# azmyrajab/polars_ols

Measured on AMD Instinct MI355X. Metric: group_regressions_per_sec, higher is better.
Workload: dtype f32

## Files before the change

### polars_ols_amd/csrc/api.hip

```cpp
#include <algorithm>
#include <cmath>
#include <cctype>
#include <cstdlib>
#include <strings.h>
#include <condition_variable>
#include <mutex>
#include <thread>

#include "common.hpp"
#include "api_internal.hpp"
#include "k1_gram_chol.hpp"
#include "k2_resident.hpp"
#include "k2w_resident.hpp"
#include "k3_rls.hpp"
#include "k4_rolling.hpp"
#include "k5_enet.hpp"
#include "k6_svd.hpp"
#include "k7_stats.hpp"
#include "k7r_robust.hpp"
#include "k7c_cluster.hpp"
#include "k7i_influence.hpp"
#include "k8_wide.hpp"
#include "k10_ridge_path.hpp"
#include "k11_rlm.hpp"
#include "k13_glm.hpp"
#include "k14_iv.hpp"
#include "k12_enet_cv.hpp"
#include "dyn_prep.hpp"

namespace pols {
template <typename T> bool k1m_fits(int k_user, bool has_w, int64_t max_rows);

__global__ void __launch_bounds__(256) mark_fallback_kernel(const int64_t *offs, int64_t n_groups, int32_t *status, int32_t *fb_flag,
                                                            int32_t epoch, int only_if_not_empty) {
    const int64_t g = (int64_t)blockIdx.x * 256 + threadIdx.x;
    if (g == 0) *fb_flag = epoch;
    if (g >= n_groups) return;
    if (only_if_not_empty) { if (status[g] != POLS_GROUP_EMPTY) status[g] = POLS_GROUP_FALLBACK; }
    else status[g] = POLS_GROUP_FALLBACK;
    (void)offs;
}

static thread_local char g_err[512] = "";

void set_error(const char *fmt, ...) {
    va_list ap;
    va_start(ap, fmt);
    vsnprintf(g_err, sizeof(g_err), fmt, ap);
    va_end(ap);
}

int fail(int code, const char *fmt, ...) {
    va_list ap;
    va_start(ap, fmt);
    vsnprintf(g_err, sizeof(g_err), fmt, ap);
    va_end(ap);
    return code;
}

int grow(DeviceBuffer &b, size_t bytes, void **out, bool *fresh) {
    if (fresh) *fresh = bytes > b.cap;
    if (bytes > b.cap) {
        if (b.ptr) POLS_HIP(hipFree(b.ptr));
        b.ptr = nullptr;
        b.cap = 0;
        const size_t want = std::max(bytes, (size_t)1 << 16);
        POLS_HIP(hipMalloc(&b.ptr, want));
        b.cap = want;
    }
    *out = b.ptr;
    return POLS_OK;
}
int grow(CachedTable &t, size_t bytes, void **out) {
    if (bytes > t.buf.cap) t.valid = false;
    return grow(t.buf, bytes, out);
}
int ensure_scratch(pols_ctx *ctx, Work w, size_t bytes, void **out) { return grow(ctx->work[(int)w], bytes, out); }

int upload_small(pols_ctx *ctx, void *dst_device, const void *src, size_t bytes) {
    if (bytes == 0) return POLS_OK;
    if (bytes > ((size_t)1 << 20)) {
        POLS_HIP(hipMemcpyAsync(dst_device, src, bytes, hipMemcpyHostToDevice, ctx->stream));
        POLS_HIP(hipStreamSynchronize(ctx->stream));
        return POLS_OK;
    }
    auto &slot = ctx->pinned[ctx->pinned_next];
    ctx->pinned_next = (ctx->pinned_next + 1) % 4;
    if (slot.busy) { POLS_HIP(hipEventSynchronize(slot.done)); slot.busy = false; }
    if (bytes > slot.cap) {
        if (slot.ptr) POLS_HIP(hipHostFree(slot.ptr));
        slot.ptr = nullptr; slot.cap = 0;
        const size_t want = std::max(bytes, (size_t)1 << 16);
        POLS_HIP(hipHostMalloc(&slot.ptr, want, hipHostMallocDefault));
        slot.cap = want;
    }
    if (!slot.done) POLS_HIP(hipEventCreateWithFlags(&slot.done, hipEventDisableTiming));
    std::memcpy(slot.ptr, src, bytes);
    POLS_HIP(hipMemcpyAsync(dst_device, slot.ptr, bytes, hipMemcpyHostToDevice, ctx->stream));
    POLS_HIP(hipEventRecord(slot.done, ctx->stream));
    slot.busy = true;
    return POLS_OK;
}

int upload_offsets(pols_ctx *ctx, const int64_t *offs, int64_t n_groups, const int64_t **d_offs, int64_t *max_rows,
                   uint64_t generation) {
    const int64_t cnt = n_groups + 1;
    const size_t bytes = sizeof(int64_t) * (size_t)cnt;
    if (generation != 0 && ctx->offsets.valid && ctx->offs_host == offs && ctx->offs_n == n_groups &&
        ctx->offs_generation == generation) {
        *d_offs = static_cast<const int64_t *>(ctx->offsets.buf.ptr);
        *max_rows = ctx->offs_max_rows;
        return POLS_OK;
    }
    uint64_t h0 = 1469598103934665603ULL, h1 = 0x9E3779B97F4A7C15ULL, h2 = 0xC2B2AE3D27D4EB4FULL, h3 = 0x165667B19E3779F9ULL;
    const uint64_t P = 1099511628211ULL;
    const uint64_t *u = reinterpret_cast<const uint64_t *>(offs);
    int64_t g = 0;
    for (; g + 4 <= cnt; g += 4) {
        h0 = (h0 ^ u[g]) * P; h1 = (h1 ^ u[g + 1]) * P; h2 = (h2 ^ u[g + 2]) * P; h3 = (h3 ^ u[g + 3]) * P;
    }
    for (; g < cnt; ++g) h0 = (h0 ^ u[g]) * P;
    int64_t mx = 0, ored = 0, mn = 0, mn_pos = INT64_MAX;
    for (int64_t i = 0; i < cnt; ++i) ored |= offs[i];
    int32_t small_mask = 0;
    int64_t hist_cnt[48] = {0}, hist_rows[48] = {0};
    int64_t over = 0;
    for (int64_t i = 1; i < cnt; ++i) {
        const int64_t d = offs[i] - offs[i - 1];
        mn = d < mn ? d : mn; mx = d > mx ? d : mx;
        mn_pos = (d > 0 && d < mn_pos) ? d : mn_pos;
        over += d > 1021 ? d - 1021 : 0;
        if (d > 0 && d <= 32) small_mask |= d <= 4 ? 1 : (d <= 8 ? 2 : (d <= 16 ? 4 : 8));
        const int bkt = d <= 1 ? 0 : 64 - __builtin_clzll((unsigned long long)(d - 1));
        hist_cnt[bkt < 47 ? bkt : 47]++; hist_rows[bkt < 47 ? bkt : 47] += d;
    }
    if (mn < 0) return fail(POLS_ERR_INVALID, "group_offsets must be ascending");
    const uint64_t sum = ((h0 * 31 + h1) * 31 + h2) * 31 + h3;
    const bool hit = ctx->offsets.valid && ctx->offs_n == n_groups && ctx->offs_sum == sum &&
                     ctx->offs_copy.size() == (size_t)cnt && std::memcmp(ctx->offs_copy.data(), offs, bytes) == 0;
    if (!hit) {
        void *dptr = nullptr;
        ctx->offsets.valid = false;
        int rc = grow(ctx->offsets, bytes, &dptr);
        if (rc) return rc;
        if ((rc = upload_small(ctx, dptr, offs, bytes))) return rc;
        ctx->offsets.valid = true;
        ctx->offs_copy.assign(offs, offs + cnt);
        ctx->offs_n = n_groups;
        ctx->offs_sum = sum;
        ctx->offs_id++;
    }
    ctx->offs_host = offs;
    ctx->offs_generation = generation;
    ctx->offs_max_rows = mx;
    ctx->offs_min_rows = mn_pos == INT64_MAX ? 0 : mn_pos;
    ctx->offs_small_mask = small_mask;
    std::memcpy(ctx->offs_hist_cnt, hist_cnt, sizeof(hist_cnt));
    std::memcpy(ctx->offs_hist_rows, hist_rows, sizeof(hist_rows));
    ctx->offs_wave_overflow = over;
    {
        int64_t tail = -1;
        for (int64_t i = n_groups; i >= 1; --i)
            if (offs[i] > offs[i - 1]) { tail = i - 1; break; }
        ctx->offs_tail_group = tail;
    }
    ctx->offs_aligned[0] = (ored & 1) == 0;
    ctx->offs_aligned[1] = (ored & 3) == 0;
    *d_offs = static_cast<const int64_t *>(ctx->offsets.buf.ptr);
    *max_rows = mx;
    return POLS_OK;
}

static bool ieq(const char *a, const char *b) {
    for (; *a && *b; ++a, ++b)
        if (std::tolower((unsigned char)*a) != std::tolower((unsigned char)*b)) return false;
    return *a == *b;
}

bool options_set(Options &o, const char *key, const char *v) {
    if (!key) return false;
    if (!strncasecmp(key, "POLS_", 5)) key += 5;
    const bool on = v != nullptr;
    const Options d;
    if (ieq(key, "TIMELINE")) o.timeline = on;
    else if (ieq(key, "K1_NOOCC4")) o.k1_noocc4 = on;
    else if (ieq(key, "K1_NOFAST")) o.k1_nofast = on;
    else if (ieq(key, "K1_NOEDGE")) o.k1_noedge = on;
    else if (ieq(key, "K1_NOTINY")) o.k1_notiny = on;
    else if (ieq(key, "K1_NORC1")) o.k1_norc1 = on;
    else if (ieq(key, "K1_SHAPE")) { o.k1_shape_team = on && ieq(v, "team"); o.k1_shape_wave = on && ieq(v, "wave"); }
    else if (ieq(key, "K1_F64_TEAM")) o.k1_f64_team256 = on && std::atoi(v) == 256;
    else if (ieq(key, "KG_NOYV")) o.kg_noyv = on;
    else if (ieq(key, "KG_SINGLE_BUFFER")) o.kg_single_buffer = on;
    else if (ieq(key, "NO_CLASSES")) o.no_classes = on;
    else if (ieq(key, "PREDICT_LOOP")) o.predict_loop = on;
    else if (ieq(key, "K2_NOPREFETCH")) o.k2_noprefetch = on;
    else if (ieq(key, "NO_SPLIT")) o.no_split = on;
    else if (ieq(key, "K1_PASSES")) o.k1_passes = on ? std::atoi(v) : d.k1_passes;
    else if (ieq(key, "K1_WG")) o.k1_wg = on ? std::atoi(v) : d.k1_wg;
    else if (ieq(key, "K1T_RC4")) o.k1t_rc4 = on ? (std::atoi(v) != 0) : d.k1t_rc4;
    else if (ieq(key, "K1T_SUB8")) o.k1t_sub8 = on ? std::atoi(v) : d.k1t_sub8;
    else if (ieq(key, "K1_NT_LOADS")) o.k1_nt_loads = on ? (std::atoi(v) != 0) : d.k1_nt_loads;
    else if (ieq(key, "K1_XCD")) o.k1_xcd = on ? std::atoi(v) : d.k1_xcd;
    else if (ieq(key, "K4P_LPS")) o.k4p_lps = on ? std::atoi(v) : d.k4p_lps;
    else if (ieq(key, "SEG_TARGET")) o.seg_target = on ? std::atoi(v) : d.seg_target;
    else if (ieq(key, "K1_RC2_WIDE")) o.k1_rc2_wide = on ? std::atoi(v) != 0 : d.k1_rc2_wide;
    else if (ieq(key, "DEBUG_SKIP_FIXUP")) o.debug_skip_fixup = on && std::atoi(v) != 0;
    else if (ieq(key, "K1_PERSIST")) o.k1_persist = on ? (std::atoi(v) != 0) : d.k1_persist;
    else if (ieq(key, "K1_PERSIST_SUB")) o.k1_persist_sub = on ? std::atoi(v) : d.k1_persist_sub;
    else if (ieq(key, "K1T_SUB32")) o.k1t_sub32 = on ? (std::atoi(v) != 0) : d.k1t_sub32;
    else if (ieq(key, "STATIC_ENGINE")) o.static_engine = !on ? 0 : ieq(v, "stream") ? 1 : ieq(v, "k2") ? 2 : ieq(v, "nok2") ? 3 : ieq(v, "k2w") ? 4 : 0;
    else if (ieq(key, "RLS_ENGINE")) o.rls_engine = !on ? 0 : ieq(v, "seq") ? 1 : ieq(v, "scan") ? 2 : ieq(v, "chunk") ? 3 : ieq(v, "halo") ? 4 : 0;
    else if (ieq(key, "RLM_ENGINE")) o.rlm_engine = !on ? 0 : ieq(v, "stream") ? 1 : 0;
    else if (ieq(key, "GLM_ENGINE")) o.glm_engine = !on ? 0 : ieq(v, "split") ? 1 : 0;
    else if (ieq(key, "RLS_SPINS")) o.rls_spin_limit = on ? std::atoi(v) : d.rls_spin_limit;
    else if (ieq(key, "RLS_EARLY")) o.rls_early = on ? std::atoi(v) : d.rls_early;
    else if (ieq(key, "ROLLING_ENGINE")) o.rolling_engine = !on ? 0 : ieq(v, "chunk") ? 1 : ieq(v, "halo") ? 2 : ieq(v, "nocompact") ? 3 : ieq(v, "halowave") ? 4 : ieq(v, "scatter") ? 5 : 0;
    else if (ieq(key, "K1_ENGINE")) o.k1_engine = !on ? 0 : ieq(v, "valu") ? 1 : ieq(v, "mfma") ? 2 : 0;
    else if (ieq(key, "K9_TAKE")) o.k9_take = !on ? 0 : ieq(v, "gather") ? 1 : ieq(v, "scatter") ? 2 : 0;
    else return false;
    return true;
}

void options_from_env(Options &o) {
    static const char *const keys[] = {"TIMELINE", "K1_NOOCC4", "K1_NOFAST", "K1_NOTINY", "K1_NORC1", "K1_SHAPE", "K1_F64_TEAM",
                                       "KG_NOYV", "K2_NOPREFETCH", "K1_PASSES", "K1_WG", "RLS_SPINS", "RLS_EARLY", "K1T_RC4", "K1_NT_LOADS", "STATIC_ENGINE",
                                       "RLS_ENGINE", "RLM_ENGINE", "GLM_ENGINE", "ROLLING_ENGINE", "K1_ENGINE", "K9_TAKE", "K1_PERSIST", "K1_PERSIST_SUB", "K1T_SUB32", "K1_NOEDGE", "K1T_SUB8",
                                       "K1_XCD", "NO_SPLIT", "DEBUG_SKIP_FIXUP", "K4P_LPS", "SEG_TARGET", "K1_RC2_WIDE", "KG_SINGLE_BUFFER", "PREDICT_LOOP", "NO_CLASSES"};
    char name[64];
    for (const char *k : keys) {
        std::snprintf(name, sizeof(name), "POLS_%s", k);
        if (const char *v = std::getenv(name)) options_set(o, k, v);
    }
}

static bool timing_sampled(pols_ctx *ctx) {
    if (!ctx->timing) return false;
    return (ctx->timing_tick++ % ctx->timing_stride) == 0;
}

void timing_begin(pols_ctx *ctx) {
    ctx->timing_open = false;
    if (!timing_sampled(ctx)) return;
    ctx->timing_open = true;
    if (ctx->timed_used == ctx->timed.size()) {
        TimedLaunch t;
        if (hipEventCreate(&t.start) != hipSuccess || hipEventCreate(&t.stop) != hipSuccess) return;
        ctx->timed.push_back(t);
    }
    hipEventRecord(ctx->timed[ctx->timed_used].start, ctx->stream);
}

bool timing_pair(pols_ctx *ctx, hipEvent_t *start, hipEvent_t *stop) {
    if (!timing_sampled(ctx)) return false;
    if (ctx->timed_used == ctx->timed.size()) {
        TimedLaunch t;
        if (hipEventCreate(&t.start) != hipSuccess || hipEventCreate(&t.stop) != hipSuccess) return false;
        ctx->timed.push_back(t);
    }
    *start = ctx->timed[ctx->timed_used].start;
    *stop = ctx->timed[ctx->timed_used].stop;
    ctx->timed_used++;
    return true;
}

void timing_end(pols_ctx *ctx) {
    if (!ctx->timing_open || ctx->timed_used >= ctx->timed.size()) return;
    ctx->timing_open = false;
    hipEventRecord(ctx->timed[ctx->timed_used].stop, ctx->stream);
    ctx->timed_used++;
}

int check_ctx(pols_ctx *ctx) {
    if (!ctx) return fail(POLS_ERR_INVALID, "ctx is NULL");
    POLS_HIP(hipSetDevice(ctx->device));
    return POLS_OK;
}


template <typename T>
__global__ void __launch_bounds__(256) null_weights_kernel(const T *w, T *out, int64_t n) {
    using V = typename Vec16<T>::type;
    constexpr int VN = Vec16<T>::N;
    const int64_t i0 = ((int64_t)blockIdx.x * 256 + threadIdx.x) * VN;
    if (i0 + VN <= n) {
        const V v = *reinterpret_cast<const V *>(w + i0);
        T f[4];
#pragma unroll
        for (int e = 0; e < VN; ++e) { const T x = vget<T>(v, e); f[e] = x != x ? (T)1e-24 : x; }
        if constexpr (VN == 4) *reinterpret_cast<V *>(out + i0) = V{f[0], f[1], f[2], f[3]};
        else *reinterpret_cast<V *>(out + i0) = V{f[0], f[1]};
    } else {
        for (int64_t i = i0; i < n; ++i) { const T x = w[i]; out[i] = x != x ? (T)1e-24 : x; }
    }
}

int fill_null_weights(pols_ctx *ctx, const pols_batch *b, Staged *st) {
    if (!st->w || b->null_free || b->n_rows <= 0) return POLS_OK;
    void *dst = const_cast<void *>(st->w);
    if (b->mem == POLS_MEM_DEVICE) {
        int rc = ensure_scratch(ctx, Work::NullWeights, round256(dtype_size(b->dtype) * (size_t)b->n_rows), &dst);
        if (rc) return rc;
    }
    const int vn = b->dtype == POLS_F32 ? 4 : 2;
    const unsigned blocks = (unsigned)((b->n_rows + 256 * (int64_t)vn - 1) / (256 * (int64_t)vn));
    if (b->dtype == POLS_F32) hipLaunchKernelGGL(null_weights_kernel<float>, dim3(blocks), dim3(256), 0, ctx->stream, static_cast<const float *>(st->w), static_cast<float *>(dst), b->n_rows);
    else hipLaunchKernelGGL(null_weights_kernel<double>, dim3(blocks), dim3(256), 0, ctx->stream, static_cast<const double *>(st->w), static_cast<double *>(dst), b->n_rows);
    POLS_HIP(hipGetLastError());
    st->w = dst;
    return POLS_OK;
}

int stage_inputs(pols_ctx *ctx, const pols_batch *b, int64_t coef_rows, int kt, const pols_out *o, Staged *st) {
    const size_t sz = dtype_size(b->dtype);
    const size_t colb = round256(sz * (size_t)b->n_rows);
    st->x.assign((size_t)b->n_features, nullptr);
    if (b->mem == POLS_MEM_DEVICE) {
        st->y = b->y; st->w = b->weights; st->valid = b->valid;
        for (int j = 0; j < b->n_features; ++j) st->x[j] = b->x_cols[j];
        if (o) { st->coef = o->coef; st->pred = o->pred; st->resid = o->resid; st->status = o->status; }
        bool ok = aligned16(st->y) && aligned16(st->w) && aligned16(st->pred) && aligned16(st->resid);
        for (int j = 0; j < b->n_features; ++j) ok = ok && aligned16(st->x[j]);
        if (!ok) return fail(POLS_ERR_INVALID, "device columns must be 16-byte aligned");
        return POLS_OK;
    }
    const int ncols = b->n_features + 1 + (b->weights ? 1 : 0);
    void *in = nullptr, *out = nullptr;
    int rc = ensure_scratch(ctx, Work::HostInputs, colb * ncols + round256((size_t)b->n_rows), &in);
    if (rc) return rc;
    char *p = static_cast<char *>(in);
    auto put = [&](const void *src, size_t bytes, const void **dst) -> int {
        POLS_HIP(hipMemcpyAsync(p, src, bytes, hipMemcpyHostToDevice, ctx->stream));
        *dst = p;
        p += round256(bytes);
        return POLS_OK;
    };
    if ((rc = put(b->y, sz * b->n_rows, &st->y))) return rc;
    for (int j = 0; j < b->n_features; ++j)
        if ((rc = put(b->x_cols[j], sz * b->n_rows, &st->x[j]))) return rc;
    if (b->weights && (rc = put(b->weights, sz * b->n_rows, &st->w))) return rc;
    if (b->valid) {
        const void *v = nullptr;
        if ((rc = put(b->valid, (size_t)b->n_rows, &v))) return rc;
        st->valid = static_cast<const uint8_t *>(v);
    }
    if (o) {
        const size_t coefb = round256(sz * (size_t)coef_rows * kt);
        const size_t statb = round256(sizeof(int32_t) * (size_t)b->n_groups);
        rc = ensure_scratch(ctx, Work::HostOutputs, coefb + 2 * colb + statb, &out);
        if (rc) return rc;
        char *q = static_cast<char *>(out);
        if (o->coef) st->coef = q;
        q += coefb;
        if (o->pred) st->pred = q;
        q += colb;
        if (o->resid) st->resid = q;
        q += colb;
        if (o->status) st->status = reinterpret_cast<int32_t *>(q);
    }
    return POLS_OK;
}

int unstage_outputs(pols_ctx *ctx, const pols_batch *b, int64_t coef_rows, int kt, const pols_out *o, const Staged &st) {
    if (b->mem == POLS_MEM_DEVICE) return POLS_OK;
    const size_t sz = dtype_size(b->dtype);
    if (o->coef) POLS_HIP(hipMemcpyAsync(o->coef, st.coef, sz * (size_t)coef_rows * kt, hipMemcpyDeviceToHost, ctx->stream));
    if (o->pred) POLS_HIP(hipMemcpyAsync(o->pred, st.pred, sz * (size_t)b->n_rows, hipMemcpyDeviceToHost, ctx->stream));
    if (o->resid) POLS_HIP(hipMemcpyAsync(o->resid, st.resid, sz * (size_t)b->n_rows, hipMemcpyDeviceToHost, ctx->stream));
    if (o->status) POLS_HIP(hipMemcpyAsync(o->status, st.status, sizeof(int32_t) * (size_t)b->n_groups, hipMemcpyDeviceToHost, ctx->stream));
    POLS_HIP(hipStreamSynchronize(ctx->stream));
    return POLS_OK;
}

int check_batch(const pols_batch *b, const pols_out *o, int max_features) {
    if (!b || !o) return fail(POLS_ERR_INVALID, "batch / out is NULL");
    if (b->dtype != POLS_F32 && b->dtype != POLS_F64) return fail(POLS_ERR_INVALID, "dtype must be POLS_F32 or POLS_F64");
    if (b->mem != POLS_MEM_HOST && b->mem != POLS_MEM_DEVICE) return fail(POLS_ERR_INVALID, "mem must be POLS_MEM_HOST or POLS_MEM_DEVICE");
    if (b->n_rows < 0 || b->n_groups < 0) return fail(POLS_ERR_INVALID, "negative size");
    if (b->n_features < 1) return fail(POLS_ERR_INVALID, "must pass at least 2 series");
    if (b->n_features + (b->add_intercept ? 1 : 0) > max_features)
        return fail(POLS_ERR_UNSUPPORTED, "%d features (+ intercept) > %d", b->n_features, max_features);
    if (!b->group_offsets || !b->x_cols || (!b->y && b->n_rows)) return fail(POLS_ERR_INVALID, "NULL column / offsets pointer");
    if (b->group_offsets[0] != 0 || b->group_offsets[b->n_groups] != b->n_rows)
        return fail(POLS_ERR_INVALID, "group_offsets must start at 0 and end at n_rows");
    for (int j = 0; j < b->n_features; ++j)
        if (!b->x_cols[j] && b->n_rows) return fail(POLS_ERR_INVALID, "x_cols[%d] is NULL", j);
    return POLS_OK;
}

static bool k1_valu_takes(const pols_ctx *ctx, bool f32, int kt, int64_t max_rows, bool has_w = false) {
    const int vec = f32 ? 4 : 2;
    if (kt <= 8 && max_rows <= (int64_t)256 * 2 * vec) return true;
    const int64_t need = max_rows + (ctx->offs_aligned[f32 ? 1 : 0] ? 0 : vec - 1);
    if (kt <= K1_MAX_KT && ctx->opt.static_engine != 2) {
        if (kt <= 8 || (ctx->opt.k1_rc2_wide && !(!f32 && kt == 10 && has_w))) return need <= (int64_t)256 * 4 * vec;
        return need <= 1024;
    }
    if (kt <= K1_MAX_KT) return need <= 1024;
    if (kt <= K1W_MAX_KT) return need <= (int64_t)256 * 2 * vec;
    if (!f32 && kt == 16 && need <= 16 * vec && !ctx->opt.k1_notiny) return true;
    if (!f32 && (kt < 17 || kt > 24)) return false;
    return kt <= K1X_MAX_KT && need <= (int64_t)256 * 1 * vec;
}
static bool k1_nulls_takes(const pols_ctx *ctx, bool f32, int kt, int64_t max_rows) {
    const int vec = f32 ? 4 : 2;
    if (kt <= 8 && max_rows <= (int64_t)256 * 2 * vec) return true;
    const int64_t need = max_rows + (ctx->offs_aligned[f32 ? 1 : 0] ? 0 : vec - 1);
    if (kt <= K1_MAX_KT) return need <= 1024;
    if (kt <= K1W_MAX_KT) return need <= (int64_t)256 * 2 * vec;
    if (!f32 && (kt < 17 || kt > 24)) return false;
    return kt <= K1X_MAX_KT && need <= (int64_t)256 * 1 * vec;
}

struct Compacted {
    pols_batch bb;
    std::vector<int64_t> offs;
    std::vector<const void *> xcols, ycols;
    Staged st;
    const int64_t *d_offs = nullptr;
    const uint8_t *vbytes = nullptr;
    RowCompactArgs ra;
};

static int compact_nulls(pols_ctx *ctx, const pols_batch *b, int policy, Compacted *c, const void *const *targets = nullptr,
                         int n_targets = 0) {
    int rc;
    const int64_t *d_offs = nullptr;
    int64_t max_rows = 0;
    Staged &st = c->st;
    if ((rc = upload_offsets(ctx, b->group_offsets, b->n_groups, &d_offs, &max_rows, b->offsets_generation))) return rc;
    if ((rc = stage_inputs(ctx, b, 0, 0, nullptr, &st))) return rc;
    const int m = n_targets > 0 ? n_targets : 1;
    const int k = b->n_features, ncols = m + k + (st.w ? 1 : 0);
    const size_t G = (size_t)b->n_groups, N = (size_t)b->n_rows;
    const size_t sz = dtype_size(b->dtype), colb = round256(sz * std::max<size_t>(N, 1));
    const size_t n_slabs = (N + 255) / 256;
    const size_t vb = round256(std::max<size_t>(N, 1)), tabb = round256(sizeof(void *) * (size_t)ncols), offb = round256(sizeof(int64_t) * (G + 1));
    const size_t cntb = round256(sizeof(uint32_t) * std::max<size_t>(n_slabs, 1)), baseb = round256(sizeof(int64_t) * (n_slabs + 1)),
                 gfb = round256(sizeof(int64_t) * std::max<size_t>(n_slabs, 1));
    void *d = nullptr;
    const bool stage_targets = n_targets > 0 && b->mem == POLS_MEM_HOST;
    if ((rc = ensure_scratch(ctx, Work::DynPrep, cntb + baseb + gfb + vb + 2 * tabb + offb + colb * (size_t)(ncols + (stage_targets ? m : 0)), &d))) return rc;
    char *base = static_cast<char *>(d);
    char *q_valid = base + cntb + baseb + gfb, *q_tab = q_valid + vb, *q_offs = q_tab + 2 * tabb;
    char *cols = q_offs + offb;
    std::vector<const void *> inp((size_t)ncols);
    std::vector<void *> outp((size_t)ncols);
    for (int t = 0; t < m; ++t) {
        const void *src = n_targets > 0 ? targets[t] : st.y;
        if (stage_targets) {
            char *dst = cols + colb * (size_t)(ncols + t);
            POLS_HIP(hipMemcpyAsync(dst, targets[t], sz * N, hipMemcpyHostToDevice, ctx->stream));
            src = dst;
        }
        inp[(size_t)t] = src;
    }
    for (int j = 0; j < k; ++j) inp[(size_t)(m + j)] = st.x[(size_t)j];
    if (st.w) inp[(size_t)(m + k)] = st.w;
    for (int j = 0; j < ncols; ++j) outp[(size_t)j] = cols + colb * (size_t)j;
    if ((rc = upload_small(ctx, q_tab, inp.data(), sizeof(void *) * (size_t)ncols))) return rc;
    if ((rc = upload_small(ctx, q_tab + tabb, outp.data(), sizeof(void *) * (size_t)ncols))) return rc;
    RowCompactArgs ra;
    std::memset(&ra, 0, sizeof(ra));
    ra.in = reinterpret_cast<const void *const *>(q_tab);
    ra.out = reinterpret_cast<void *const *>(q_tab + tabb);
    ra.n_cols = ncols;
    ra.w_col = st.w ? m + k : -1;
    ra.drop = (policy == POLS_NULL_DROP || policy == POLS_NULL_DROP_ZERO || policy == POLS_NULL_DROP_WINDOW || policy == POLS_NULL_DROP_Y_ZERO_X) ? 1 : 0;
    ra.n_mask = policy == POLS_NULL_DROP_Y_ZERO_X ? m : m + k;
    ra.zero_fill = (policy == POLS_NULL_ZERO || policy == POLS_NULL_DROP_Y_ZERO_X) ? 1 : 0;
    ra.valid_in = st.valid;
    ra.valid_out = reinterpret_cast<uint8_t *>(q_valid);
    ra.valid = ra.valid_out;
    ra.offs = d_offs; ra.n_rows = (int64_t)N; ra.n_groups = b->n_groups; ra.n_slabs = (int64_t)n_slabs;
    ra.slab_cnt = reinterpret_cast<uint32_t *>(base);
    ra.slab_base = reinterpret_cast<int64_t *>(base + cntb);
    ra.slab_gfirst = reinterpret_cast<int64_t *>(base + cntb + baseb);
    ra.c_offs = reinterpret_cast<int64_t *>(q_offs);
    c->offs.assign(G + 1, 0);
    if (N > 0) {
        if ((rc = row_compact_mask_launch(ctx, b->dtype, ra))) return rc;
        if ((rc = row_compact_offsets_launch(ctx, ra))) return rc;
        POLS_HIP(hipMemcpyAsync(c->offs.data(), ra.c_offs, sizeof(int64_t) * (G + 1), hipMemcpyDeviceToHost, ctx->stream));
        POLS_HIP(hipStreamSynchronize(ctx->stream));
        if ((rc = row_compact_scatter_launch(ctx, b->dtype, ra))) return rc;
    }
    struct { uint8_t *vbytes; } ca{ra.valid_out};
    c->ra = ra;
    c->xcols.assign(outp.begin() + m, outp.begin() + m + k);
    c->ycols.assign(outp.begin(), outp.begin() + m);
    c->d_offs = d_offs;
    c->vbytes = ca.vbytes;
    c->bb = *b;
    c->bb.mem = POLS_MEM_DEVICE;
    c->bb.n_rows = c->offs[G];
    c->bb.group_offsets = c->offs.data();
    c->bb.offsets_generation = 0;
    c->bb.y = outp[0];
    c->bb.x_cols = c->xcols.data();
    c->bb.weights = st.w ? outp[(size_t)(m + k)] : nullptr;
    c->bb.valid = nullptr;
    c->bb.null_free = 1;
    return POLS_OK;
}

}

using namespace pols;

extern "C" {

int pols_device_count(void) {
    int n = 0;
    if (hipGetDeviceCount(&n) != hipSuccess) return 0;
    return n;
}

const char *pols_version(void) { return "pols_mi355x 0.1.0 (gfx950)"; }
const char *pols_last_error(void) { return g_err; }

int pols_create(int device_id, pols_ctx **out) {
    if (!out) return fail(POLS_ERR_INVALID, "out is NULL");
    *out = nullptr;
    int n = 0;
    if (hipGetDeviceCount(&n) != hipSuccess || n <= 0)
        return fail(POLS_ERR_NO_DEVICE, "no HIP device visible; libpols_mi355x has no CPU fallback");
    if (device_id < 0 || device_id >= n) return fail(POLS_ERR_INVALID, "device_id %d out of range [0, %d)", device_id, n);
    POLS_HIP(hipSetDevice(device_id));
    hipDeviceProp_t prop;
    POLS_HIP(hipGetDeviceProperties(&prop, device_id));
    if (std::strncmp(prop.gcnArchName, "gfx950", 6) != 0)
// ... 260 lines not shown
    const bool hit = same_frame && sc.nz2 >= extra_per_seg;
    auto lay = [&](char *sb, int64_t n_seg) {
        const size_t b_so = round256(sizeof(int64_t) * (size_t)(ids ? 2 * n_seg : n_seg + 1)), b_sm = round256(sizeof(int32_t) * (size_t)n_seg),
                     b_sf = round256(sizeof(int32_t) * (size_t)(n_items + 1));
        t->offs = reinterpret_cast<const int64_t *>(sb);
        t->map = reinterpret_cast<const int32_t *>(sb + b_so);
        t->first = reinterpret_cast<const int32_t *>(sb + b_so + b_sm);
        t->extra = sb + b_so + b_sm + b_sf;
        t->n_seg = n_seg;
        return b_so + b_sm + b_sf;
    };
    if (hit) { lay(static_cast<char *>(sc.buf.ptr), sc.n_seg); t->max_len = sc.max_len; t->max_seg = sc.max_seg; return POLS_OK; }
    if (same_frame) extra_per_seg = std::max<size_t>(extra_per_seg, sc.nz2);
    sc.valid = false;
    std::vector<int64_t> so;
    std::vector<int32_t> sm, sf((size_t)n_items + 1);
    if (!ids) so.push_back(0);
    int64_t max_len = 0, max_seg = 0;
    for (int64_t i = 0; i < n_items; ++i) {
        const int64_t g = ids ? (int64_t)(*ids)[(size_t)i] : i;
        if (i > 0) max_seg = std::max<int64_t>(max_seg, (int64_t)sm.size() - sf[(size_t)i - 1]);
        sf[(size_t)i] = (int32_t)sm.size();
        const int64_t s0 = b->group_offsets[g], e0 = b->group_offsets[g + 1];
        const int64_t pieces = std::max<int64_t>(1, (e0 - s0 + seg_target - 1) / seg_target);
        const int64_t len = std::max<int64_t>(1, ((e0 - s0 + pieces - 1) / pieces + 255) / 256 * 256);
        max_len = std::max(max_len, std::min(len, e0 - s0));
        for (int64_t r = s0; r < e0 || r == s0; r += len) {
            if (ids) so.push_back(r);
            so.push_back(std::min(e0, r + len));
            sm.push_back((int32_t)i);
            if (e0 == s0) break;
        }
    }
    sf[(size_t)n_items] = (int32_t)sm.size();
    if (n_items > 0) max_seg = std::max<int64_t>(max_seg, (int64_t)sm.size() - sf[(size_t)n_items - 1]);
    const int64_t n_seg = (int64_t)sm.size();
    const size_t tabs = round256(sizeof(int64_t) * so.size()) + round256(sizeof(int32_t) * sm.size()) + round256(sizeof(int32_t) * sf.size());
    void *ds = nullptr;
    if ((rc = grow(sc, tabs + round256(extra_per_seg * (size_t)n_seg), &ds))) return rc;
    char *sb = static_cast<char *>(ds);
    lay(sb, n_seg);
    if ((rc = upload_small(ctx, const_cast<int64_t *>(t->offs), so.data(), sizeof(int64_t) * so.size()))) return rc;
    if ((rc = upload_small(ctx, const_cast<int32_t *>(t->map), sm.data(), sizeof(int32_t) * sm.size()))) return rc;
    if ((rc = upload_small(ctx, const_cast<int32_t *>(t->first), sf.data(), sizeof(int32_t) * sf.size()))) return rc;
    sc.valid = true; sc.offs_id = ctx->offs_id; sc.n_groups = b->n_groups; sc.n_rows = b->n_rows; sc.seg_target = seg_target;
    sc.class_key = class_key; sc.n_items = n_items;
    sc.n_seg = n_seg; sc.nz2 = extra_per_seg; sc.nulls = false; sc.max_len = max_len; sc.max_seg = max_seg;
    t->max_len = max_len; t->max_seg = max_seg;
    return POLS_OK;
}

static int pick_size_classes(const pols_ctx *ctx, bool f32, int64_t n_groups, int64_t max_rows, int64_t (&t)[2]) {
    t[0] = t[1] = 0;
    if (ctx->opt.no_classes || n_groups < 2048) return 0;
    const double alpha = 0.5, launch_cost = 6.0e5;
    const int b0 = f32 ? 7 : 6;
    int bc = b0;
    while (((int64_t)1 << bc) < max_rows && bc < 46) ++bc;
    auto cost = [&](int s0, int s1) {
        double c = launch_cost * ((s0 >= 0) + (s1 >= 0));
        for (int q = 0; q < 48; ++q) {
            if (!ctx->offs_hist_cnt[q]) continue;
            const double avg = (double)ctx->offs_hist_rows[q] / (double)ctx->offs_hist_cnt[q];
            const int kb = (s0 >= 0 && q <= s0) ? s0 : ((s1 >= 0 && q <= s1) ? s1 : bc);
            c += (double)ctx->offs_hist_cnt[q] * std::max(avg, alpha * (double)((int64_t)1 << kb));
        }
        return c;
    };
    auto count_le = [&](int sb) { int64_t n = 0; for (int q = 0; q <= sb; ++q) n += ctx->offs_hist_cnt[q]; return n; };
    const double one = cost(-1, -1);
    double best = one;
    int bs0 = -1, bs1 = -1;
    for (int s1 = b0; s1 < bc; ++s1) {
        const int64_t le1 = count_le(s1);
        if (le1 == 0 || le1 == n_groups) continue;
        const double c1 = cost(-1, s1);
        if (c1 < best) { best = c1; bs0 = -1; bs1 = s1; }
        for (int s0 = b0; s0 < s1; ++s0) {
            const int64_t le0 = count_le(s0);
            if (le0 == 0 || le0 == le1) continue;
            const double c2 = cost(s0, s1);
            if (c2 < 0.9 * c1 && c2 < best) { best = c2; bs0 = s0; bs1 = s1; }
        }
    }
    if (bs1 < 0 || !(best < 0.75 * one)) return 0;
    const int slack = ctx->offs_aligned[f32 ? 1 : 0] ? 0 : (f32 ? 3 : 1);
    int n = 0;
    if (bs0 >= 0) t[n++] = ((int64_t)1 << bs0) - slack;
    t[n++] = ((int64_t)1 << bs1) - slack;
    return n;
}

static int ls_core(pols_ctx *ctx, const pols_batch *b, const pols_ols_params *p, pols_out *o, LsInfo *info) {
    int rc = check_ctx(ctx);
    if (rc) return rc;
    if ((rc = check_batch(b, o, K8_KMAX))) return rc;
    if (!p) return fail(POLS_ERR_INVALID, "params is NULL");
    if (p->null_policy < POLS_NULL_IGNORE || p->null_policy > POLS_NULL_DROP_WINDOW) return fail(POLS_ERR_INVALID, "unknown null_policy %d", p->null_policy);
    const int pol = (b->null_free && !b->valid) ? POLS_NULL_IGNORE : p->null_policy;
    const bool nulls = pol != POLS_NULL_IGNORE;
    if (b->valid && (pol == POLS_NULL_IGNORE || pol == POLS_NULL_ZERO))
        return fail(POLS_ERR_INVALID, "a validity mask needs a drop-family null_policy");

    const int m = p->solve_method;
    const double alpha = p->alpha;
    const bool positive = p->positive != 0;
    double ridge_alpha = 0.0, enet_l1 = 0.5;
    bool enet = false;
    if (alpha == 0.0 && !positive && (m == POLS_SOLVE_AUTO || m == POLS_SOLVE_SVD || m == POLS_SOLVE_QR)) {
        ridge_alpha = 0.0;
    } else if (alpha >= 0.0 && (p->has_l1_ratio ? p->l1_ratio : 0.0) == 0.0 && !positive) {
        if (!(m == POLS_SOLVE_AUTO || m == POLS_SOLVE_CHOL || m == POLS_SOLVE_LU || m == POLS_SOLVE_SVD))
            return fail(POLS_ERR_PANIC, "Only 'Cholesky', 'LU', & 'SVD' are currently supported solver methods for Ridge.");
        ridge_alpha = alpha;
    } else {
        if (!(m == POLS_SOLVE_AUTO || m == POLS_SOLVE_CD || m == POLS_SOLVE_CD_ACTIVE_SET))
            return fail(POLS_ERR_PANIC, "Only solve_method 'CD' (coordinate descent) is currently supported for Elastic Net / Lasso problems.");
        if (!(alpha > 0.0)) return fail(POLS_ERR_PANIC, "'alpha' must be strictly positive");
        const double l1 = p->has_l1_ratio ? p->l1_ratio : 0.5;
        if (!(l1 >= 0.0 && l1 <= 1.0)) return fail(POLS_ERR_PANIC, "'l1_ratio' must be strictly between 0. and 1.");
        enet = true;
        enet_l1 = l1;
    }

    const int kt = b->n_features + (b->add_intercept ? 1 : 0);
    if (b->n_groups == 0) return POLS_OK;
    if (kt > 31) {
        const bool ols_b = !enet && ridge_alpha == 0.0 && alpha == 0.0 && (m == POLS_SOLVE_AUTO || m == POLS_SOLVE_SVD || m == POLS_SOLVE_QR);
        if (info) return fail(POLS_ERR_INVALID, "internal: the wide statistics path calls wide_static itself");
        return wide_static(ctx, b, p, o, kt, enet, ridge_alpha, enet_l1, ols_b);
    }
    const int64_t *d_offs = nullptr;
    int64_t max_rows = 0;
    if ((rc = upload_offsets(ctx, b->group_offsets, b->n_groups, &d_offs, &max_rows, b->offsets_generation))) return rc;
    Staged st;
    if ((rc = stage_inputs(ctx, b, b->n_groups, kt, o, &st))) return rc;
    if ((rc = fill_null_weights(ctx, b, &st))) return rc;
    auto finish = [&](double *gram) -> int {
        if (!info) return unstage_outputs(ctx, b, b->n_groups, kt, o, st);
        info->st = st; info->d_offs = d_offs; info->max_rows = max_rows; info->gram = gram; info->kt = kt;
        return POLS_OK;
    };
    if (!enet && !st.status) {
        void *sp = nullptr;
        if ((rc = ensure_scratch(ctx, Work::Status, sizeof(int32_t) * (size_t)b->n_groups, &sp))) return rc;
        st.status = static_cast<int32_t *>(sp);
    }
    if (!enet) {
        if (!ctx->fb_flag) {
            POLS_HIP(hipMalloc(reinterpret_cast<void **>(&ctx->fb_flag), 256));
            POLS_HIP(hipMemsetAsync(ctx->fb_flag, 0, 256, ctx->stream));
        }
        ctx->epoch = (ctx->epoch % 0x0ffffff0) + 1;
    }
    const bool ols_branch = !enet && ridge_alpha == 0.0 && (m == POLS_SOLVE_AUTO || m == POLS_SOLVE_SVD || m == POLS_SOLVE_QR) && alpha == 0.0;
    const double chol_noise = 16.0 * (double)kt * 2.220446049250313e-16;
    const double pivot_tol = ols_branch ? (b->dtype == POLS_F32 ? 1e-3 : 1e-10) : (b->dtype == POLS_F32 && m != POLS_SOLVE_SVD ? 1e-3 : chol_noise);
    K6Args ka;
    int fix_workers = 0;
    auto prepare_fix = [&](int max_workers = 0) -> int {
        if (max_workers <= 0) max_workers = (int)std::max<int64_t>(64, std::min<int64_t>(2048, b->n_groups / 128));
        const int workers = (int)std::min<int64_t>(b->n_groups, max_workers);
        const int64_t stride = std::max<int64_t>(1, max_rows) * (kt + 1);
        void *wk = nullptr;
        int w_use = workers;
        while (w_use > 1 && (double)w_use * (double)stride * 8.0 > 4e9) w_use /= 2;
        int r2;
        if ((r2 = ensure_scratch(ctx, Work::Fixup, sizeof(double) * (size_t)w_use * (size_t)stride, &wk))) return r2;
        std::memset(&ka, 0, sizeof(ka));
        ka.y = st.y; ka.w = st.w;
        for (int j = 0; j < b->n_features; ++j) ka.x[j] = st.x[j];
        ka.offs = d_offs; ka.n_groups = b->n_groups; ka.status = st.status;
        ka.fb_flag = ctx->fb_flag; ka.epoch = ctx->epoch;
        ka.coef = st.coef; ka.pred = st.pred; ka.resid = st.resid;
        ka.work = static_cast<double *>(wk); ka.work_stride = stride;
        ka.alpha = ridge_alpha;
        ka.rc_factor = ols_branch ? 8.0 * 2.220446049250313e-16 : ((m == POLS_SOLVE_SVD && p->has_rcond) ? p->rcond : -1.0);
        ka.mode = ols_branch ? (m == POLS_SOLVE_AUTO ? FIX_OLS_AUTO : m == POLS_SOLVE_QR ? FIX_OLS_QR : FIX_MINNORM)
                             : (m == POLS_SOLVE_SVD ? FIX_MINNORM : m == POLS_SOLVE_LU ? FIX_LU : FIX_CHOL_LU);
        ka.k_user = b->n_features; ka.kt = kt;
        ka.valid = st.valid; ka.null_policy = pol;
        fix_workers = w_use;
        return POLS_OK;
    };
    auto svd_fixup = [&]() -> int {
        if (enet) return POLS_OK;
        if (ctx->opt.debug_skip_fixup) return POLS_OK;
        int r2 = prepare_fix();
        if (r2) return r2;
        return k6_launch(ctx, b->dtype, ka, fix_workers);
    };

    const bool tiny_frame = !enet && b->n_rows < (b->dtype == POLS_F32 ? 4 : 2);
    if (!enet && ((!ols_branch && m == POLS_SOLVE_SVD && p->has_rcond) || tiny_frame)) {
        if ((rc = prepare_fix(2048))) return rc;
        hipLaunchKernelGGL(mark_fallback_kernel, dim3((unsigned)((b->n_groups + 255) / 256)), dim3(256), 0, ctx->stream, d_offs,
                           b->n_groups, st.status, ctx->fb_flag, ctx->epoch, 0);
        POLS_HIP(hipGetLastError());
        ctx->last_kernel = "k6_small_svd_all_groups";
        if ((rc = k6_launch(ctx, b->dtype, ka, fix_workers))) return rc;
        return finish(nullptr);
    }

    {
        const bool f32 = b->dtype == POLS_F32;
        const int vec = f32 ? 4 : 2;
        const bool aligned = ctx->offs_aligned[f32 ? 1 : 0];
        const bool k2_ok = !nulls && kt <= K2_KMAX && k2_fits(b->dtype, kt, max_rows, aligned) && b->n_rows >= vec && ctx->opt.static_engine != 1 &&
                           ctx->opt.static_engine != 3;
        const bool k1_resident = nulls ? k1_nulls_takes(ctx, f32, kt, max_rows) : k1_valu_takes(ctx, f32, kt, max_rows, b->weights != nullptr);
        const int64_t k2_cap = max_rows > (int64_t)512 * 2 * vec ? (int64_t)512 * 4 * vec : (int64_t)512 * 2 * vec;
        const bool k2_sparse = !enet && ctx->opt.static_engine != 2 && max_rows > (int64_t)256 * 2 * vec && b->n_groups >= 2048 &&
                               (double)b->n_rows < 0.3 * (double)k2_cap * (double)b->n_groups;
        const bool legacy_forced = (ctx->opt.k1_engine == 2 && kt <= K1M_MAX_KT) || (ctx->opt.k1_engine == 1 && kt <= K1_MAX_KT);
        (void)K1W_MAX_KT;
        const bool k1m_takes = kt <= K1M_MAX_KT && (f32 ? k1m_fits<float>(b->n_features, b->weights != nullptr, max_rows)
                                                        : k1m_fits<double>(b->n_features, b->weights != nullptr, max_rows));
        const bool k1m_wins = k1m_takes && f32 && kt >= 9 && kt <= 10;
        const bool want = enet || m == POLS_SOLVE_LU || ctx->opt.static_engine == 2 || (!k1_resident && !legacy_forced && !k1m_wins);
        if (k2_ok && want && !k2_sparse) {
            K2Args a2;
            std::memset(&a2, 0, sizeof(a2));
            a2.y = st.y; a2.w = st.w;
            for (int j = 0; j < K2_KMAX; ++j) a2.x[j] = j < b->n_features ? st.x[j] : st.y;
            a2.offs = d_offs; a2.n_groups = b->n_groups; a2.n_rows = b->n_rows;
            a2.coef = st.coef; a2.pred = st.pred; a2.resid = st.resid; a2.status = st.status;
            a2.k_user = b->n_features; a2.kt = kt;
            a2.solver = enet ? (m == POLS_SOLVE_CD_ACTIVE_SET ? K2_CD_ACTIVE_SET : K2_CD) : (m == POLS_SOLVE_LU ? K2_LU : K2_CHOL);
            a2.lu_fallback = (!enet && !ols_branch && m != POLS_SOLVE_SVD) ? 1 : 0;
            a2.alpha = enet ? alpha : ridge_alpha;
            a2.l1_ratio = enet_l1; a2.tol = p->tol; a2.max_iter = p->max_iter; a2.positive = positive ? 1 : 0;
            a2.pivot_tol = a2.lu_fallback ? chol_noise : pivot_tol;
            a2.fb_flag = enet ? nullptr : ctx->fb_flag; a2.epoch = ctx->epoch;
            if ((rc = k2_launch(ctx, b->dtype, a2, max_rows))) return rc;
            if ((rc = svd_fixup())) return rc;
            return finish(nullptr);
        }
    }

    {
        const bool f32 = b->dtype == POLS_F32;
        const int vec = f32 ? 4 : 2;
        const bool fits = !enet && !nulls && m != POLS_SOLVE_LU && k2w_fits(b->dtype, kt, max_rows, ctx->offs_aligned[f32 ? 1 : 0]) && b->n_rows >= vec &&
                          ctx->opt.static_engine != 1 && ctx->opt.static_engine != 3;
        const bool k1_resident = k1_valu_takes(ctx, f32, kt, max_rows);
        const bool short_wide = !f32 && (max_rows > 256 ? kt >= 24 : (kt >= 23 || (kt == 22 && max_rows >= 192) || (kt >= 20 && max_rows >= 224)));
        if (fits && (!k1_resident || short_wide || ctx->opt.static_engine == 4)) {
            K2wArgs aw;
            std::memset(&aw, 0, sizeof(aw));
            aw.y = st.y; aw.w = st.w;
            for (int j = 0; j < 32; ++j) aw.x[j] = j < b->n_features ? st.x[j] : st.y;
            aw.offs = d_offs; aw.n_groups = b->n_groups; aw.n_rows = b->n_rows;
            aw.coef = st.coef; aw.pred = st.pred; aw.resid = st.resid; aw.status = st.status;
            aw.k_user = b->n_features; aw.kt = kt;
            aw.alpha = ridge_alpha; aw.pivot_tol = pivot_tol;
            aw.fb_flag = ctx->fb_flag; aw.epoch = ctx->epoch;
            if ((rc = k2w_launch(ctx, b->dtype, aw, max_rows))) return rc;
            if ((rc = svd_fixup())) return rc;
            return finish(nullptr);
        }
    }

    bool stream = enet;
    if (!enet) {
        const bool f32 = b->dtype == POLS_F32;
        const bool fits_lds = f32 ? k1m_fits<float>(b->n_features, b->weights != nullptr, max_rows)
                                  : k1m_fits<double>(b->n_features, b->weights != nullptr, max_rows);
        const bool k1_resident = nulls ? k1_nulls_takes(ctx, f32, kt, max_rows) : k1_valu_takes(ctx, f32, kt, max_rows, b->weights != nullptr);
        stream = (nulls && !k1_resident) || (!k1_resident && (kt > K1M_MAX_KT || !fits_lds));
        const bool k5v_ok = !nulls && kt <= K5V_MAX_KT && !ctx->opt.kg_single_buffer && ctx->opt.k1_engine == 0;
        stream = stream || (!k1_resident && k5v_ok);
        stream = stream || ctx->opt.static_engine == 1;
        stream = stream || (m == POLS_SOLVE_LU && kt > K1M_MAX_KT);
    }
    double *stream_gram = nullptr;
    auto run_stream = [&](const std::vector<int32_t> *ids, const int32_t *d_ids, int64_t class_key, int64_t cls_max_rows) -> int {
        const int64_t ng = ids ? (int64_t)ids->size() : b->n_groups;
        const int64_t mr = ids ? cls_max_rows : max_rows;
        void *scr = nullptr;
        const size_t nz = (size_t)kt + 1;
        const size_t gram_bytes = round256(sizeof(double) * nz * nz * (size_t)ng);
        const size_t c64_bytes = round256(sizeof(double) * (size_t)kt * (size_t)ng);
        const size_t nv_bytes = nulls ? round256(sizeof(double) * (size_t)b->n_groups) : 0;
        SegTables sg;
        if ((rc = ensure_segments(ctx, b, mr, sizeof(double) * (nz * nz + 1), &sg, ids, class_key))) return rc;
        const bool split = sg.n_seg > 0;
        const int n_slices = (split && sg.max_seg >= 256 && ng <= 256) ? 16 : 1;
        const size_t slice_bytes = n_slices > 1 ? round256(sizeof(double) * nz * nz * (size_t)n_slices * (size_t)ng) : 0;
        if ((rc = ensure_scratch(ctx, Work::Gram, gram_bytes + c64_bytes + nv_bytes + slice_bytes, &scr))) return rc;
        double *nvalid = nulls ? reinterpret_cast<double *>(static_cast<char *>(scr) + gram_bytes + c64_bytes) : nullptr;
        const int64_t *seg_offs = split ? sg.offs : d_offs;
        const int32_t *seg_map = sg.map, *seg_first = sg.first;
        const int64_t n_seg = split ? sg.n_seg : ng;
        double *gram_part = reinterpret_cast<double *>(sg.extra);
        double *nv_part = (split && nulls) ? gram_part + nz * nz * (size_t)n_seg : nullptr;
        GramArgs ga;
        std::memset(&ga, 0, sizeof(ga));
        ga.y = st.y; ga.w = st.w;
        for (int j = 0; j < b->n_features; ++j) ga.x[j] = st.x[j];
        ga.offs = seg_offs; ga.n_groups = n_seg; ga.n_rows = b->n_rows; ga.offs_pairs = ids ? 1 : 0;
        ga.gram = split ? gram_part : static_cast<double *>(scr);
        ga.k_user = b->n_features; ga.kt = kt;
        ga.valid = st.valid; ga.null_policy = pol; ga.nvalid = split ? nv_part : nvalid;
        if ((rc = gram_stream_launch(ctx, b->dtype, ga))) return rc;
        if (split) {
            GramReduceArgs ra;
            std::memset(&ra, 0, sizeof(ra));
            ra.part = gram_part; ra.nv_part = nv_part; ra.first = seg_first;
            ra.gram = static_cast<double *>(scr); ra.nvalid = nvalid; ra.n_groups = ng; ra.nz2 = (int32_t)(nz * nz);
            ra.max_segments = (int32_t)std::min<int64_t>(1 << 30, sg.max_seg);
            if (n_slices > 1) { ra.slices = reinterpret_cast<double *>(static_cast<char *>(scr) + gram_bytes + c64_bytes + nv_bytes); ra.n_slices = n_slices; }
            if ((rc = gram_reduce_launch(ctx, ra))) return rc;
            ga.gram = static_cast<double *>(scr);
            ctx->last_kernel += "_split";
        }
        CdArgs ca;
        std::memset(&ca, 0, sizeof(ca));
        ca.gram = ga.gram; ca.offs = d_offs; ca.n_groups = ng; ca.glist = d_ids;
        ca.coef = st.coef; ca.coef64 = reinterpret_cast<double *>(static_cast<char *>(scr) + gram_bytes);
        ca.status = st.status;
        ca.alpha = alpha; ca.l1_ratio = enet_l1; ca.tol = p->tol; ca.max_iter = p->max_iter;
        ca.positive = positive ? 1 : 0; ca.active_set = (m == POLS_SOLVE_CD_ACTIVE_SET) ? 1 : 0; ca.kt = kt;
        ca.nvalid = nvalid;
        if (enet) {
            if ((rc = gram_cd_launch(ctx, b->dtype, ca))) return rc;
        } else {
            ca.alpha = ridge_alpha;
            ca.solver = (m == POLS_SOLVE_LU) ? 1 : 0;
            ca.lu_fallback = (!ols_branch && m != POLS_SOLVE_SVD) ? 1 : 0;
            ca.pivot_tol = ca.lu_fallback ? chol_noise : pivot_tol;
            ca.fb_flag = ctx->fb_flag; ca.epoch = ctx->epoch;
            if ((rc = gram_solve_launch(ctx, b->dtype, ca))) return rc;
        }
        if (st.pred || st.resid) {
            PredictArgs pa;
            std::memset(&pa, 0, sizeof(pa));
            pa.y = st.y; pa.w = st.w;
            for (int j = 0; j < b->n_features; ++j) pa.x[j] = st.x[j];
            pa.offs = seg_offs; pa.n_groups = n_seg; pa.n_rows = b->n_rows; pa.gmap = seg_map; pa.offs_pairs = ids ? 1 : 0;
            pa.max_item_rows = split ? sg.max_len : mr;
            pa.coef64 = ca.coef64; pa.pred = st.pred; pa.resid = st.resid;
            pa.k_user = b->n_features; pa.kt = kt;
            pa.valid = st.valid; pa.null_policy = pol;
            if ((rc = predict_launch(ctx, b->dtype, pa))) return rc;
        }
        stream_gram = ga.gram;
        return POLS_OK;
    };

    K1Args a;
    std::memset(&a, 0, sizeof(a));
    a.y = st.y; a.w = st.w; a.valid = st.valid;
    for (int j = 0; j < b->n_features; ++j) a.x[j] = st.x[j];
    a.offs = d_offs;
    a.n_groups = b->n_groups;
    a.n_rows = b->n_rows;
    a.coef = st.coef; a.pred = st.pred; a.resid = st.resid; a.status = st.status;
    a.alpha = ridge_alpha;
    a.pivot_tol = pivot_tol;
    a.fb_flag = ctx->fb_flag; a.epoch = ctx->epoch;
    a.k_user = b->n_features;
    a.null_policy = pol;
    const bool f32b = b->dtype == POLS_F32;
    auto k1_takes = [&](int64_t rows) { return nulls ? k1_nulls_takes(ctx, f32b, kt, rows) : k1_valu_takes(ctx, f32b, kt, rows, b->weights != nullptr); };
    const bool classes_allowed = !enet && !ctx->opt.no_classes && !ctx->opt.timeline && ctx->opt.k1_persist <= 0 && ctx->opt.static_engine == 0 &&
                                 ctx->opt.k1_engine == 0 && b->n_groups >= 2048 && b->n_groups <= 0x7fffffffLL && m != POLS_SOLVE_LU;
    auto build_lists = [&](const int64_t *cut, int n_cut) -> int {
        auto &cc = ctx->class_cache;
        bool same = cc.valid && cc.offs_id == ctx->offs_id && cc.n_cut == n_cut;
        for (int c = 0; c < n_cut && same; ++c) same = cc.cut[c] == cut[c];
        if (same) return POLS_OK;
        cc.valid = false;
        std::vector<int32_t> lists[4];
        for (int64_t g = 0; g < b->n_groups; ++g) {
            const int64_t n = b->group_offsets[g + 1] - b->group_offsets[g];
            int c = 0;
            while (c < n_cut && n > cut[c]) ++c;
            lists[c].push_back((int32_t)g);
        }
        void *d = nullptr;
        int r2 = grow(cc, sizeof(int32_t) * (size_t)b->n_groups, &d);
        if (r2) return r2;
        size_t at = 0;
        for (int c = 0; c <= n_cut; ++c) {
            if (!lists[c].empty() && (r2 = upload_small(ctx, static_cast<int32_t *>(d) + at, lists[c].data(), sizeof(int32_t) * lists[c].size()))) return r2;
            cc.n[c] = (int64_t)lists[c].size();
            at += lists[c].size();
        }
        for (int c = n_cut + 1; c < 4; ++c) cc.n[c] = 0;
        cc.host_last.swap(lists[n_cut]);
        cc.valid = true; cc.offs_id = ctx->offs_id; cc.n_cut = n_cut;
        for (int c = 0; c < n_cut; ++c) cc.cut[c] = cut[c];
        return POLS_OK;
    };
    auto launch_k1_classes = [&](const int64_t *cut, int n_cut, int c_lo, int c_hi, std::string &names) -> int {
        const auto &cc = ctx->class_cache;
        int64_t first[4] = {0, cc.n[0], cc.n[0] + cc.n[1], cc.n[0] + cc.n[1] + cc.n[2]};
        for (int c = c_hi; c >= c_lo; --c) {
            if (cc.n[c] == 0) continue;
            K1Args ac = a;
            ac.glist = static_cast<const int32_t *>(cc.buf.ptr) + first[c];
            ac.n_groups = cc.n[c];
            ac.class_max_rows = c < n_cut ? cut[c] : max_rows;
            int r2 = k1_launch(ctx, b->dtype, kt, ac, ac.class_max_rows, true);
            if (r2) return r2;
            names += (names.empty() ? "" : " | ") + ctx->last_kernel;
        }
        return POLS_OK;
    };

    if (stream) {
        int64_t k1_top = 0;
        if (classes_allowed && !k1_takes(max_rows)) {
            const int slack = ctx->offs_aligned[f32b ? 1 : 0] ? 0 : (f32b ? 3 : 1);
            for (int bb = 13; bb >= (f32b ? 7 : 6) && k1_top == 0; --bb)
                if (((int64_t)1 << bb) - slack < max_rows && k1_takes(((int64_t)1 << bb) - slack)) k1_top = ((int64_t)1 << bb) - slack;
            int64_t rows_low = 0;
            for (int q = 0; q < 48 && k1_top > 0; ++q)
                if (((int64_t)1 << q) <= k1_top + 3) rows_low += ctx->offs_hist_rows[q];
            if ((double)rows_low < 0.3 * (double)b->n_rows) k1_top = 0;
        }
        if (k1_top > 0) {
            int64_t cut[3];
            int64_t low_t[2];
            const int n_low = pick_size_classes(ctx, f32b, b->n_groups, k1_top, low_t);
            int n_cut = 0;
            for (int c = 0; c < n_low; ++c) cut[n_cut++] = low_t[c];
            cut[n_cut++] = k1_top;
            if ((rc = build_lists(cut, n_cut))) return rc;
            if ((rc = prepare_fix())) return rc;
            std::string names;
            const auto &cc = ctx->class_cache;
            if (cc.n[n_cut] > 0) {
                const int32_t *d_top = static_cast<const int32_t *>(cc.buf.ptr) + (b->n_groups - cc.n[n_cut]);
                if ((rc = run_stream(&cc.host_last, d_top, k1_top, max_rows))) return rc;
                names = ctx->last_kernel;
            }
            if ((rc = launch_k1_classes(cut, n_cut, 0, n_cut - 1, names))) return rc;
            ctx->last_kernel = names;
            if ((rc = k6_launch(ctx, b->dtype, ka, fix_workers))) return rc;
            return finish(nullptr);
        }
        if ((rc = run_stream(nullptr, nullptr, 0, 0))) return rc;
        if ((rc = svd_fixup())) return rc;
        return finish(stream_gram);
    }

    if ((rc = prepare_fix())) return rc;
    int64_t class_t[2];
    const int n_cut = (classes_allowed && k1_takes(max_rows)) ? pick_size_classes(ctx, f32b, b->n_groups, max_rows, class_t) : 0;
    if (n_cut > 0) {
        if ((rc = build_lists(class_t, n_cut))) return rc;
        std::string names;
        if ((rc = launch_k1_classes(class_t, n_cut, 0, n_cut, names))) return rc;
        ctx->last_kernel = names;
    } else {
        if ((rc = k1_launch(ctx, b->dtype, kt, a, max_rows, true))) return rc;
    }
    if ((rc = k6_launch(ctx, b->dtype, ka, fix_workers))) return rc;
    return finish(nullptr);
}

int pols_least_squares(pols_ctx *ctx, const pols_batch *b, const pols_ols_params *p, pols_out *o) {
    return ls_core(ctx, b, p, o, nullptr);
}

int pols_multi_target_least_squares(pols_ctx *ctx, const pols_batch *b, const void *const *y_cols, int32_t n_targets,
                                    const pols_ols_params *p, void *const *pred_cols, void *coef, int32_t *status) {
    int rc = check_ctx(ctx);
    if (rc) return rc;
    if (!b || !p || !y_cols) return fail(POLS_ERR_INVALID, "batch / params / y_cols is NULL");
    if (n_targets < 1 || n_targets > 256) return fail(POLS_ERR_INVALID, "n_targets must be in 1..256");
    for (int t = 0; t < n_targets; ++t)
        if (!y_cols[t] || (pred_cols && !pred_cols[t])) return fail(POLS_ERR_INVALID, "target / prediction column %d is NULL", t);
    pols_batch bb = *b;
    bb.y = y_cols[0];
    pols_out o;
    std::memset(&o, 0, sizeof(o));
    o.coef = coef; o.status = status;
    if ((rc = check_batch(&bb, &o, K8_KMAX))) return rc;
    const double l1 = p->has_l1_ratio ? p->l1_ratio : 0.0;
    if (p->positive || l1 != 0.0)
        return fail(POLS_ERR_PANIC, "Multi-target regression is only supported for unconstrained OLS & Ridge problems.");
    if (!(p->solve_method == POLS_SOLVE_AUTO || p->solve_method == POLS_SOLVE_SVD))
        return fail(POLS_ERR_PANIC, "only solve_method='svd' is supported for multi-target regressions");
    if (!(p->alpha >= 0.0)) return fail(POLS_ERR_PANIC, "alpha must be non-negative");
    if (p->null_policy < POLS_NULL_IGNORE || p->null_policy > POLS_NULL_DROP_WINDOW) return fail(POLS_ERR_INVALID, "unknown null_policy %d", p->null_policy);
    if (b->valid && (p->null_policy == POLS_NULL_IGNORE || p->null_policy == POLS_NULL_ZERO))
        return fail(POLS_ERR_INVALID, "a validity mask needs a drop-family null_policy");
    const int kt = b->n_features + (b->add_intercept ? 1 : 0);
    if (kt + n_targets > K8_KMAX) return fail(POLS_ERR_UNSUPPORTED, "%d columns + %d targets > %d", kt, n_targets, K8_KMAX);
    if (b->n_groups == 0) return POLS_OK;
    const int policy = p->null_policy == POLS_NULL_IGNORE ? POLS_NULL_ZERO : p->null_policy;
    if (!b->null_free || b->valid) {
        Compacted c;
        if ((rc = compact_nulls(ctx, &bb, policy, &c, y_cols, n_targets))) return rc;
        const bool host = b->mem == POLS_MEM_HOST;
        const size_t G = (size_t)b->n_groups, N = (size_t)b->n_rows, sz = dtype_size(b->dtype);
        const size_t coefb = round256(sz * G * n_targets * kt), statb = round256(sizeof(int32_t) * G), colb = round256(sz * std::max<size_t>(N, 1));
        const size_t tabb = round256(sizeof(void *) * (size_t)std::max(b->n_features, n_targets));
        void *d = nullptr;
        if ((rc = ensure_scratch(ctx, Work::CompactOut, coefb + statb + 2 * tabb + (host && pred_cols ? colb * (size_t)n_targets : 0), &d))) return rc;
        char *q = static_cast<char *>(d);
        void *dcoef = (!host && coef) ? coef : static_cast<void *>(q);
        int32_t *dstat = (!host && status) ? status : reinterpret_cast<int32_t *>(q + coefb);
        char *tabs = q + coefb + statb, *preds = tabs + 2 * tabb;
        pols_ols_params pp = *p;
        pp.null_policy = POLS_NULL_IGNORE;
        if ((rc = pols_multi_target_least_squares(ctx, &c.bb, c.ycols.data(), n_targets, &pp, nullptr, dcoef, dstat))) return rc;
        if (pred_cols) {
            const int64_t *d_offs = nullptr;
            int64_t mr = 0;
            if ((rc = upload_offsets(ctx, b->group_offsets, b->n_groups, &d_offs, &mr, b->offsets_generation))) return rc;
            std::vector<void *> pt((size_t)n_targets);
            for (int t = 0; t < n_targets; ++t) pt[(size_t)t] = host ? static_cast<void *>(preds + colb * (size_t)t) : pred_cols[t];
            if ((rc = upload_small(ctx, tabs, c.st.x.data(), sizeof(void *) * (size_t)b->n_features))) return rc;
            if ((rc = upload_small(ctx, tabs + tabb, pt.data(), sizeof(void *) * (size_t)n_targets))) return rc;
            MtPredictArgs ma;
            std::memset(&ma, 0, sizeof(ma));
            ma.xtab = reinterpret_cast<const void *const *>(tabs);
            ma.ptab = reinterpret_cast<void *const *>(tabs + tabb);
            ma.w = c.st.w; ma.coef = dcoef; ma.vbytes = c.vbytes; ma.offs = d_offs; ma.n_groups = b->n_groups;
            ma.k_user = b->n_features; ma.kt = kt; ma.m = n_targets;
            ma.mask_drop = p->null_policy == POLS_NULL_DROP ? 1 : 0;
            ma.row_blocks = (int32_t)std::min<int64_t>(1024, std::max<int64_t>(1, (int64_t)(N / std::max<size_t>(G, 1)) / 4096));
            if ((rc = mt_predict_launch(ctx, b->dtype, ma))) return rc;
            if (host)
                for (int t = 0; t < n_targets; ++t)
                    POLS_HIP(hipMemcpyAsync(pred_cols[t], pt[(size_t)t], sz * N, hipMemcpyDeviceToHost, ctx->stream));
        }
        if (host) {
            if (coef) POLS_HIP(hipMemcpyAsync(coef, dcoef, sz * G * n_targets * kt, hipMemcpyDeviceToHost, ctx->stream));
            if (status) POLS_HIP(hipMemcpyAsync(status, dstat, sizeof(int32_t) * G, hipMemcpyDeviceToHost, ctx->stream));
            POLS_HIP(hipStreamSynchronize(ctx->stream));
        }
        return POLS_OK;
    }
    return wide_static(ctx, &bb, p, &o, kt, false, p->alpha, 0.0, p->alpha == 0.0, y_cols, n_targets, pred_cols);
}

static int cluster_device_ids(pols_ctx *ctx, const pols_batch *b, const pols_cluster_params *cl, int ways, const int64_t **dev) {
    if (b->mem == POLS_MEM_DEVICE) {
        for (int w = 0; w < ways; ++w) dev[w] = cl->ids[w];
        return POLS_OK;
    }
    const size_t colb = round256(sizeof(int64_t) * (size_t)std::max<int64_t>(b->n_rows, 1));
    void *d = nullptr;
    int rc = ensure_scratch(ctx, Work::ClusterIds, colb * (size_t)ways, &d);
    if (rc) return rc;
    for (int w = 0; w < ways; ++w) {
        char *dst = static_cast<char *>(d) + colb * (size_t)w;
        if (b->n_rows) POLS_HIP(hipMemcpyAsync(dst, cl->ids[w], sizeof(int64_t) * (size_t)b->n_rows, hipMemcpyHostToDevice, ctx->stream));
        dev[w] = reinterpret_cast<const int64_t *>(dst);
    }
    return POLS_OK;
}

struct InflCall {
    const pols_influence_params *q;
    const pols_influence_out *io;
    bool rows_by_caller = false;
    double *prep = nullptr, *grp = nullptr;
};

static int influence_rows(pols_ctx *ctx, const pols_batch *b, const Staged &st, const int64_t *d_offs, const SegTables &sg, const uint8_t *valid,
                          int zero_fill, const InflCall &ic) {
    const bool host = b->mem == POLS_MEM_HOST;
    const size_t G = (size_t)b->n_groups, N = (size_t)b->n_rows, sz = dtype_size(b->dtype), colb = round256(sz * std::max<size_t>(N, 1));
    const pols_influence_out *io = ic.io;
    void *const user[K7I_NOUT] = {io->leverage, io->student_internal, io->student_external, io->cooks_d, io->dffits, io->se_mean,
                                  io->se_obs, io->mean_lo, io->mean_hi, io->obs_lo, io->obs_hi};
    int rc, n_out = 0;
    for (int i = 0; i < K7I_NOUT; ++i) n_out += user[i] ? 1 : 0;
    InflArgs a;
    std::memset(&a, 0, sizeof(a));
    a.y = st.y; a.w = st.w;
    for (int j = 0; j < b->n_features; ++j) a.x[j] = st.x[(size_t)j];
    a.offs = d_offs; a.n_groups = b->n_groups; a.n_rows = b->n_rows;
    if (sg.n_seg > 0) { a.seg_offs = sg.offs; a.seg_map = sg.map; a.n_seg = sg.n_seg; }
    a.valid = valid; a.zero_fill = zero_fill;
    a.k_user = b->n_features; a.kt = b->n_features + (b->add_intercept ? 1 : 0);
    a.prep = ic.prep; a.grp = ic.grp;
    void *rows = nullptr;
    if (host && n_out && (rc = ensure_scratch(ctx, Work::InflRows, colb * (size_t)n_out, &rows))) return rc;
    char *q = static_cast<char *>(rows);
    for (int i = 0; i < K7I_NOUT; ++i) {
        if (!user[i]) continue;
        if (!host && !aligned16(user[i])) return fail(POLS_ERR_INVALID, "device columns must be 16-byte aligned");
        a.out[i] = host ? static_cast<void *>(q) : user[i];
        q += host ? colb : 0;
    }
    if ((rc = k7i_rows_launch(ctx, b->dtype, a))) return rc;
    if (host && N)
        for (int i = 0; i < K7I_NOUT; ++i)
            if (user[i]) POLS_HIP(hipMemcpyAsync(user[i], a.out[i], sz * N, hipMemcpyDeviceToHost, ctx->stream));
    double *const gu[3] = {io->sigma2, io->df, io->t_crit};
    for (int i = 0; i < 3; ++i)
        if (gu[i]) POLS_HIP(hipMemcpyAsync(gu[i], ic.grp + (size_t)i * G, sizeof(double) * G, host ? hipMemcpyDeviceToHost : hipMemcpyDeviceToDevice, ctx->stream));
    return POLS_OK;
}

static int statistics_body(pols_ctx *ctx, const pols_batch *b, const pols_ols_params *p, const pols_cov_params *cov,
                           const pols_cluster_params *cl, pols_out *o, const pols_stats_out *s, InflCall *infl = nullptr) {
    int rc = check_ctx(ctx);
    if (rc) return rc;
    if ((rc = check_batch(b, o, K8_KMAX))) return rc;
    if (!p || !s) return fail(POLS_ERR_INVALID, "params / stats is NULL");
    if (p->null_policy < POLS_NULL_IGNORE || p->null_policy > POLS_NULL_DROP_WINDOW) return fail(POLS_ERR_INVALID, "unknown null_policy %d", p->null_policy);
    if (b->valid && (p->null_policy == POLS_NULL_IGNORE || p->null_policy == POLS_NULL_ZERO))
        return fail(POLS_ERR_INVALID, "a validity mask needs a drop-family null_policy");
    if (b->n_groups == 0) return POLS_OK;
    if ((p->null_policy != POLS_NULL_IGNORE && !b->null_free) || b->valid) {
        Compacted c;
        if ((rc = compact_nulls(ctx, b, p->null_policy, &c))) return rc;
        pols_ols_params pp = *p;
        pp.null_policy = POLS_NULL_IGNORE;
        const size_t G = (size_t)b->n_groups, sz = dtype_size(b->dtype);
        pols_cluster_params cc;
        if (cl) {
            cc = *cl;
            const int ways = cl->cov_type == POLS_COV_CLUSTER2 ? 2 : 1;
            const int64_t *src[2] = {nullptr, nullptr};
            if ((rc = cluster_device_ids(ctx, b, cl, ways, src))) return rc;
            const int64_t nv = c.offs[G];
            const size_t mapb = round256(sizeof(int32_t) * (size_t)std::max<int64_t>(nv, 1)), colb = round256(sizeof(int64_t) * (size_t)std::max<int64_t>(nv, 1));
            void *d = nullptr;
            if ((rc = ensure_scratch(ctx, Work::ClusterCompact, mapb + colb * (size_t)ways, &d))) return rc;
            int64_t *dst[2] = {nullptr, nullptr};
            for (int w = 0; w < ways; ++w) dst[w] = reinterpret_cast<int64_t *>(static_cast<char *>(d) + mapb + colb * (size_t)w);
            if (nv > 0) {
                RowCompactArgs ra = c.ra;
                ra.src = static_cast<int32_t *>(d);
                if ((rc = row_compact_srcmap_launch(ctx, ra))) return rc;
                if ((rc = k7c_gather_ids_launch(ctx, ra.src, nv, src, dst, ways))) return rc;
            }
// ... 1253 lines not shown
```

### polars_ols_amd/csrc/common.hpp

```cpp
#pragma once

#include <hip/hip_runtime.h>
#include <hip/hip_ext.h>

#include <atomic>
#include <cstdarg>
#include <cstdint>
#include <cstdio>
#include <cstring>
#include <string>
#include <vector>

#include "../../include/pols_mi355x.h"

namespace pols {

void set_error(const char *fmt, ...);
int fail(int code, const char *fmt, ...);

#define POLS_HIP(call)                                                                       \
    do {                                                                                     \
        hipError_t e_ = (call);                                                              \
        if (e_ != hipSuccess)                                                                \
            return ::pols::fail(POLS_ERR_HIP, "%s failed: %s (%s:%d)", #call, hipGetErrorString(e_), \
                                __FILE__, __LINE__);                                         \
    } while (0)

struct DeviceBuffer {
    void *ptr = nullptr;
    size_t cap = 0;
};

struct CachedTable {
    DeviceBuffer buf;
    bool valid = false;
};

enum class Work : int {
    HostInputs,
    HostOutputs,
    Fixup,
    HostStaged,
    Gram,
    Tables,
    Status,
    K3cRecords,
    K9Keys,
    Timeline,
    Arrow,
    Collective,
    DynPrep,
    CompactOut,
    NullWeights,
    RowCompact,
    CompactCoef,
    CompactStarts,
    CompactTiles,
    CompactTotals,
    GatherMap,
    RobustPrep,
    RobustMeat,
    ClusterIds,
    ClusterCompact,
    ClusterPrep,
    ClusterPart,
    ClusterSort,
    ClusterOrder,
    ClusterCounts,
    InflPrep,
    InflGroup,
    InflRows,
    RidgeCvGram,
    RidgeCvScores,
    RidgeCvOut,
    RlmCoef,
    RlmRows,
    RlmOut,
    EnetCvGram,
    EnetCvWork,
    EnetCvOut,
    GlmCoef,
    GlmState,
    GlmOffset,
    GlmOut,
    IvMoments,
    IvState,
    IvInputs,
    IvOut,
    Count
};

struct TimedLaunch {
    hipEvent_t start, stop;
};

struct Options {
    bool timeline = false;
    bool k1_noocc4 = false;
    bool k1_nofast = false;
    bool k1_notiny = false;
    bool k1_norc1 = false;
    bool k1_shape_team = false;
    bool k1_shape_wave = false;
    bool k1_f64_team256 = false;
    bool no_classes = false;
    bool kg_single_buffer = false;
    bool predict_loop = false;
    bool kg_noyv = false;
    int k1_passes = 0;
    int k1t_rc4 = -1;
    int k1t_sub8 = -1;
    int static_engine = 0;
    int rls_engine = 0;
    int rls_early = 0;
    int rls_spin_limit = -1;
    int rolling_engine = 0;
    int k1_engine = 0;
    int k9_take = 0;
    int k1_nt_loads = -1;
    bool no_split = false;
    bool k2_noprefetch = false;
    bool k1_noedge = false;
    int k1t_sub32 = -1;
    int k1_persist_sub = 0;
    int k1_persist = -1;
    bool debug_skip_fixup = false;
    bool k1_rc2_wide = true;
    int seg_target = 0;
    int k4p_lps = 0;
    int k1_wg = 0;
    int rlm_engine = 0;
    int glm_engine = 0;
    int k1_xcd = 0;
};
void options_from_env(Options &o);
bool options_set(Options &o, const char *key, const char *value);

}

struct pols_ctx {
    int device = 0;
    hipStream_t own_stream = nullptr;
    hipStream_t stream = nullptr;
    hipEvent_t switch_event = nullptr;
    int num_cus = 0;
    pols::DeviceBuffer work[(int)pols::Work::Count];
    pols::Options opt;
    bool timing = false;
    int timing_stride = 1;
    int timing_tick = 0;
    bool timing_open = false;
    std::vector<pols::TimedLaunch> timed;
    size_t timed_used = 0;
    std::string last_kernel;
    pols::CachedTable offsets;
    const int64_t *offs_host = nullptr;
    uint64_t offs_generation = 0;
    std::vector<int64_t> offs_copy;
    int64_t offs_n = -1;
    uint64_t offs_sum = 0;
    uint64_t offs_id = 0;
    struct PinnedSlot { void *ptr = nullptr; size_t cap = 0; hipEvent_t done = nullptr; bool busy = false; };
    PinnedSlot pinned[4];
    int pinned_next = 0;
    int64_t offs_max_rows = 0;
    int64_t offs_min_rows = 0;
    int64_t offs_hist_cnt[48] = {0}, offs_hist_rows[48] = {0};
    int32_t offs_small_mask = 0;
    int64_t offs_tail_group = -1;
    int64_t offs_wave_overflow = 0;
    int32_t *fb_flag = nullptr;
    int32_t epoch = 0;
    bool offs_aligned[2] = {false, false};
    struct : pols::CachedTable { uint64_t offs_id = 0; int64_t n_groups = -1, n_rows = -1, mp = -1, n_chunks = 0; int32_t chunk_len = 0;
                                 size_t b_groups = 0; } chunk_cache;
    struct : pols::CachedTable { uint64_t offs_id = 0; int64_t n_groups = -1, n_rows = -1, tile_rows = 0, n_tiles = 0; } k3c;
    struct : pols::CachedTable { uint64_t offs_id = 0; int64_t n_groups = -1, n_rows = -1, tile_rows = 0; } k3h;
    struct : pols::CachedTable { uint64_t offs_id = 0; int64_t cut[3] = {0, 0, 0}, n[4] = {0, 0, 0, 0}; int n_cut = 0;
                                 std::vector<int32_t> host_last; } class_cache;
    struct : pols::CachedTable { uint64_t offs_id = 0; int64_t n_groups = -1, n_rows = -1, seg_target = 0, n_seg = 0, max_len = 0, max_seg = 0, class_key = 0, n_items = 0; size_t nz2 = 0; bool nulls = false; } seg_cache[2];
    struct : pols::CachedTable { uint64_t offs_id = 0; int64_t n_groups = -1, n_rows = -1; } start_flags;
    pols::DeviceBuffer k3c_gran;
    unsigned long long k3c_epoch = 0;
    pols::DeviceBuffer k4c_fix;
    uint64_t k4c_fix_turn = 0;
};

namespace pols {

int grow(DeviceBuffer &b, size_t bytes, void **out, bool *fresh = nullptr);
int grow(CachedTable &t, size_t bytes, void **out);
int ensure_scratch(pols_ctx *ctx, Work w, size_t bytes, void **out);
int upload_offsets(pols_ctx *ctx, const int64_t *offs, int64_t n_groups, const int64_t **d_offs, int64_t *max_rows,
                   uint64_t generation = 0);
int upload_small(pols_ctx *ctx, void *dst_device, const void *src, size_t bytes);
void timing_begin(pols_ctx *ctx);
void timing_end(pols_ctx *ctx);
bool timing_pair(pols_ctx *ctx, hipEvent_t *start, hipEvent_t *stop);
int report_timeline(pols_ctx *ctx, const unsigned long long *d_dbg, int64_t n_groups, int n_stamps, const char *name);

inline size_t dtype_size(int dtype) { return dtype == POLS_F32 ? 4 : 8; }
inline size_t round256(size_t b) { return (b + 255) & ~(size_t)255; }

struct OncePerDevice {
    std::atomic<uint64_t> mask{0};
    bool needed(int device) const { return (mask.load(std::memory_order_acquire) & (1ull << (device & 63))) == 0; }
    void done(int device) { mask.fetch_or(1ull << (device & 63), std::memory_order_release); }
};

#if defined(__HIPCC__)

template <int CTRL, int ROW_MASK>
__device__ __forceinline__ int dpp_mov(int v) {
    return __builtin_amdgcn_update_dpp(0, v, CTRL, ROW_MASK, 0xf, false);
}

template <int CTRL, int ROW_MASK = 0xf>
__device__ __forceinline__ float dpp_get(float v) {
    return __int_as_float(dpp_mov<CTRL, ROW_MASK>(__float_as_int(v)));
}

template <int CTRL, int ROW_MASK = 0xf>
__device__ __forceinline__ double dpp_get(double v) {
    const long long b = __double_as_longlong(v);
    const int lo = dpp_mov<CTRL, ROW_MASK>((int)(b & 0xffffffffLL));
    const int hi = dpp_mov<CTRL, ROW_MASK>((int)(b >> 32));
    return __longlong_as_double(((long long)hi << 32) | (unsigned int)lo);
}

template <typename T>
__device__ __forceinline__ T wave_sum_row3(T v) {
    v += dpp_get<0xB1>(v);
    v += dpp_get<0x4E>(v);
    v += dpp_get<0x141>(v);
    v += dpp_get<0x140>(v);
    v += dpp_get<0x142, 0xa>(v);
    v += dpp_get<0x143, 0xc>(v);
    return v;
}

__device__ __forceinline__ void pair_halves(float &a, float b) {
    const auto r = __builtin_amdgcn_permlane32_swap(__float_as_uint(a), __float_as_uint(b), false, false);
    a = __uint_as_float(r[0]) + __uint_as_float(r[1]);
}
__device__ __forceinline__ void pair_halves(double &a, double b) {
    const unsigned long long ba = __double_as_longlong(a), bb = __double_as_longlong(b);
    const auto lo = __builtin_amdgcn_permlane32_swap((unsigned)ba, (unsigned)bb, false, false);
    const auto hi = __builtin_amdgcn_permlane32_swap((unsigned)(ba >> 32), (unsigned)(bb >> 32), false, false);
    a = __longlong_as_double(((unsigned long long)hi[0] << 32) | lo[0]) +
        __longlong_as_double(((unsigned long long)hi[1] << 32) | lo[1]);
}
__device__ __forceinline__ void pair_rows(float &a, float b) {
    const auto r = __builtin_amdgcn_permlane16_swap(__float_as_uint(a), __float_as_uint(b), false, false);
    a = __uint_as_float(r[0]) + __uint_as_float(r[1]);
}
__device__ __forceinline__ void pair_rows(double &a, double b) {
    const unsigned long long ba = __double_as_longlong(a), bb = __double_as_longlong(b);
    const auto lo = __builtin_amdgcn_permlane16_swap((unsigned)ba, (unsigned)bb, false, false);
    const auto hi = __builtin_amdgcn_permlane16_swap((unsigned)(ba >> 32), (unsigned)(bb >> 32), false, false);
    a = __longlong_as_double(((unsigned long long)hi[0] << 32) | lo[0]) +
        __longlong_as_double(((unsigned long long)hi[1] << 32) | lo[1]);
}
template <typename T>
__device__ __forceinline__ T row_allreduce(T v) {
    v += dpp_get<0xB1>(v);
    v += dpp_get<0x4E>(v);
    v += dpp_get<0x141>(v);
    v += dpp_get<0x140>(v);
    return v;
}

__device__ __forceinline__ constexpr int rs_perm(int row) { return row == 1 ? 2 : (row == 2 ? 1 : row); }

template <typename T, int N>
__device__ __forceinline__ void wave_reduce_scatter(T (&v)[N], T (&u)[(N + 3) / 4]) {
    constexpr int N2 = (N + 1) / 2, N4 = (N + 3) / 4;
#pragma unroll
    for (int i = 0; i < N2; ++i) {
        const T b = (2 * i + 1 < N) ? v[2 * i + 1] : T(0);
        pair_halves(v[2 * i], b);
    }
#pragma unroll
    for (int i = 0; i < N4; ++i) {
        T a = v[4 * i];
        const T b = (2 * i + 1 < N2) ? v[4 * i + 2] : T(0);
        pair_rows(a, b);
        u[i] = row_allreduce(a);
    }
}

__device__ __forceinline__ float readlane63(float v) {
    return __int_as_float(__builtin_amdgcn_readlane(__float_as_int(v), 63));
}
__device__ __forceinline__ double readlane63(double v) {
    const long long b = __double_as_longlong(v);
    const int lo = __builtin_amdgcn_readlane((int)(b & 0xffffffffLL), 63);
    const int hi = __builtin_amdgcn_readlane((int)(b >> 32), 63);
    return __longlong_as_double(((long long)hi << 32) | (unsigned int)lo);
}

__device__ __forceinline__ bool null_checks_x(int policy) {
    return policy == POLS_NULL_DROP || policy == POLS_NULL_DROP_ZERO || policy == POLS_NULL_DROP_WINDOW;
}
__device__ __forceinline__ bool null_checks_y(int policy) {
    return null_checks_x(policy) || policy == POLS_NULL_DROP_Y_ZERO_X;
}
template <typename T>
__device__ __forceinline__ bool null_row_in_fit(int policy, const uint8_t *valid, const void *y, const void *const *x, int ku, int64_t r) {
    if (policy == POLS_NULL_IGNORE || policy == POLS_NULL_ZERO) return true;
    if (valid && !valid[r]) return false;
    const T yv = static_cast<const T *>(y)[r];
    if (yv != yv) return false;
    if (null_checks_x(policy))
        for (int j = 0; j < ku; ++j) { const T v = static_cast<const T *>(x[j])[r]; if (v != v) return false; }
    return true;
}
template <typename T> __device__ __forceinline__ T nan_if(unsigned cond, T v);
template <> __device__ __forceinline__ float nan_if<float>(unsigned cond, float v) {
    return __uint_as_float(cond ? 0x7fc00000u : __float_as_uint(v));
}
template <> __device__ __forceinline__ double nan_if<double>(unsigned cond, double v) {
    return __longlong_as_double(cond ? 0x7ff8000000000000LL : __double_as_longlong(v));
}
template <typename T>
__device__ __forceinline__ T null_fill(int policy, T v) { return (policy != POLS_NULL_IGNORE && v != v) ? T(0) : v; }

template <typename T> struct Vec16;
template <> struct Vec16<float> { using type = float4; static constexpr int N = 4; };
template <> struct Vec16<double> { using type = double2; static constexpr int N = 2; };

__device__ __forceinline__ void store_stream(float4 *dst, const float4 &v) {
    __builtin_nontemporal_store(v.x, &dst->x); __builtin_nontemporal_store(v.y, &dst->y);
    __builtin_nontemporal_store(v.z, &dst->z); __builtin_nontemporal_store(v.w, &dst->w);
}
__device__ __forceinline__ void store_stream(double2 *dst, const double2 &v) {
    __builtin_nontemporal_store(v.x, &dst->x); __builtin_nontemporal_store(v.y, &dst->y);
}

__device__ __forceinline__ float4 load_stream(const float4 *p) {
    using F = __attribute__((ext_vector_type(4))) float;
    const F v = __builtin_nontemporal_load(reinterpret_cast<const F *>(p));
    return float4{v.x, v.y, v.z, v.w};
}
__device__ __forceinline__ double2 load_stream(const double2 *p) {
    using D = __attribute__((ext_vector_type(2))) double;
    const D v = __builtin_nontemporal_load(reinterpret_cast<const D *>(p));
    return double2{v.x, v.y};
}

template <typename T> __device__ __forceinline__ T vget(const typename Vec16<T>::type &v, int i);
template <> __device__ __forceinline__ float vget<float>(const float4 &v, int i) {
    return i == 0 ? v.x : i == 1 ? v.y : i == 2 ? v.z : v.w;
}
template <> __device__ __forceinline__ double vget<double>(const double2 &v, int i) { return i == 0 ? v.x : v.y; }

#endif

}
```

### polars_ols_amd/csrc/k5_enet.hip

```cpp
#include "k5_enet.hpp"
#include "k1m_kernel.inl"

namespace pols {

constexpr int KG_CR = 256;

template <typename T, int NT, bool HAS_W, bool YV = false>
__global__ void __launch_bounds__(256) gram_stream_kernel(const GramArgs a, const int rs, const int ncols, const int tile_elems, const int nbuf, const int cr) {
    using V = typename Vec16<T>::type;
    using M = Mfma16<T>;
    using acc_t = typename M::acc_t;
    constexpr int VEC = Vec16<T>::N;
    constexpr int RPP = 64 * VEC;
    constexpr int NPAIR = NT * (NT + 1) / 2;

    extern __shared__ __attribute__((aligned(16))) unsigned char smem[];
    T *const tile0 = reinterpret_cast<T *>(smem);
    T *zeros = tile0 + (size_t)nbuf * tile_elems;
    T *ones = zeros + K1M_CONST_ELEMS;

    const int tid = threadIdx.x, lane = tid & 63;
    const int wave = __builtin_amdgcn_readfirstlane(tid >> 6);
    const int64_t g = blockIdx.x;
    const int64_t s = a.offs_pairs ? a.offs[2 * g] : a.offs[g], e = a.offs_pairs ? a.offs[2 * g + 1] : a.offs[g + 1];
    const int64_t base = s - (s % VEC);
    const int head = (int)(s - base);
    const int64_t span = e - base;
    const int ku = a.k_user, kt = a.kt, NZ = kt + 1;
    const bool icpt = ku != kt;

    const int zc = lane & 15, kq = lane >> 4;
    const int rlane = (sizeof(T) == 4) ? 2 * kq : kq;
    int zsrc[NT];
#pragma unroll
    for (int t = 0; t < NT; ++t) {
        const int z = 16 * t + zc;
        if (z < ku) zsrc[t] = z;
        else if (icpt && z == kt - 1) zsrc[t] = HAS_W ? ku + 1 : -2;
        else if (z == kt) zsrc[t] = ku;
        else zsrc[t] = -1;
    }
    const bool need11 = (NT == 2) && (NZ > 17);

    acc_t acc[NPAIR][2];
#pragma unroll
    for (int p = 0; p < NPAIR; ++p) { acc[p][0] = acc_t{0, 0, 0, 0}; acc[p][1] = acc_t{0, 0, 0, 0}; }
    T xy0 = T(0), xy1 = T(0);
    double accd[NPAIR][4], xyd = 0.0;
#pragma unroll
    for (int p = 0; p < NPAIR; ++p) { accd[p][0] = 0.0; accd[p][1] = 0.0; accd[p][2] = 0.0; accd[p][3] = 0.0; }

    if (tid < 2 * K1M_CONST_ELEMS) zeros[tid] = (tid < K1M_CONST_ELEMS) ? T(0) : T(1);
    __shared__ int nfit_s;
    if (tid == 0) nfit_s = 0;
    int nfit = 0;
    const int pol = a.null_policy;
    const int nld = (HAS_W && !a.w) ? ncols - 1 : ncols;

    auto stage = [&](const int64_t c0, T *const tl) __attribute__((always_inline)) {
        const int rows_here = (int)min((int64_t)cr, span - c0);
        const int ppc = (rows_here + RPP - 1) / RPP;
        for (int p = wave; p < nld * ppc; p += 4) {
            const int col = p / ppc, q = p - col * ppc;
            const T *src = static_cast<const T *>(col < ku ? a.x[col] : (col == ku ? a.y : a.w));
            const int row0 = q * RPP + lane * VEC;
            const int64_t grow = base + c0 + row0;
            T *ldst = tl + (size_t)col * rs + q * RPP;
            if (row0 < rows_here) {
                if (grow + VEC <= a.n_rows) {
                    __builtin_amdgcn_global_load_lds((const __attribute__((address_space(1))) void *)(src + grow),
                                                     (__attribute__((address_space(3))) void *)ldst, 16, 0, 0);
                } else {
#pragma unroll
                    for (int v = 0; v < VEC; ++v) ldst[lane * VEC + v] = (grow + v < a.n_rows) ? src[grow + v] : T(0);
                }
            }
        }
    };
    if (nbuf == 2 && span > 0) stage(0, tile0);
    int buf = 0;
    for (int64_t c0 = 0; c0 < span; c0 += cr, buf ^= (nbuf - 1)) {
        const int rows_here = (int)min((int64_t)cr, span - c0);
        const int rows8 = (rows_here + 7) & ~7;
        T *const tile = tile0 + (size_t)buf * tile_elems;
        if (nbuf == 1) stage(c0, tile);
        asm volatile("s_waitcnt vmcnt(0)" ::: "memory");
        __syncthreads();
        if (nbuf == 2 && c0 + cr < span) stage(c0 + cr, tile0 + (size_t)(buf ^ 1) * tile_elems);
        const int64_t lo = head - c0, hi = span - c0;
        if constexpr (HAS_W) {
            T *wc = tile + (size_t)(ku + 1) * rs;
            for (int row0 = tid * VEC; row0 < rows8; row0 += 256 * VEC) {
                V wv;
                if (a.w) wv = *reinterpret_cast<V *>(wc + row0);
                T sw[VEC];
                bool ok[VEC];
#pragma unroll
                for (int v = 0; v < VEC; ++v) { const int r = row0 + v; ok[v] = (r >= lo && r < hi); sw[v] = a.w ? sqrt(vget<T>(wv, v)) : T(1); }
                if (pol != POLS_NULL_IGNORE) {
                    if (a.valid && null_checks_y(pol)) {
#pragma unroll
                        for (int v = 0; v < VEC; ++v) if (ok[v]) ok[v] = a.valid[base + c0 + row0 + v] != 0;
                    }
                    const int c_lo = null_checks_x(pol) ? 0 : ku, c_hi = null_checks_y(pol) ? ku : -1;
                    for (int c = c_lo; c <= c_hi; ++c) {
                        const V xv = *reinterpret_cast<V *>(tile + (size_t)c * rs + row0);
#pragma unroll
                        for (int v = 0; v < VEC; ++v) { const T x = vget<T>(xv, v); ok[v] = ok[v] && (x == x); }
                    }
                }
#pragma unroll
                for (int v = 0; v < VEC; ++v) { if (!ok[v]) sw[v] = T(0); else ++nfit; }
                if constexpr (VEC == 4) wv = V{sw[0], sw[1], sw[2], sw[3]}; else wv = V{sw[0], sw[1]};
                *reinterpret_cast<V *>(wc + row0) = wv;
                for (int c = 0; c <= ku; ++c) {
                    V xv = *reinterpret_cast<V *>(tile + (size_t)c * rs + row0);
                    T t[VEC];
#pragma unroll
                    for (int v = 0; v < VEC; ++v) t[v] = ok[v] ? null_fill<T>(pol, vget<T>(xv, v)) * sw[v] : T(0);
                    if constexpr (VEC == 4) xv = V{t[0], t[1], t[2], t[3]}; else xv = V{t[0], t[1]};
                    *reinterpret_cast<V *>(tile + (size_t)c * rs + row0) = xv;
                }
            }
            __syncthreads();
        } else {
            const int nhead = (c0 == 0) ? head : 0;
            const int ntail = rows8 - rows_here;
            const int npad = nhead + ntail;
            for (int i = tid; i < npad * ncols; i += 256) {
                const int c = i / npad, k = i - c * npad;
                const int r = (k < nhead) ? k : rows_here + (k - nhead);
                tile[(size_t)c * rs + r] = T(0);
            }
            if (npad > 0) __syncthreads();
        }
        const int nsteps = rows8 >> 3;
        const int per_wave = (nsteps + 3) >> 2;
        const int t_begin = min(nsteps, wave * per_wave), t_end = min(nsteps, t_begin + per_wave);
        const T *zp[NT];
        int zinc[NT];
#pragma unroll
        for (int t = 0; t < NT; ++t) {
            if (zsrc[t] >= 0) { zp[t] = tile + (size_t)zsrc[t] * rs + t_begin * 8 + rlane; zinc[t] = 8; }
            else { zp[t] = (zsrc[t] == -2) ? ones : zeros; zinc[t] = 0; }
        }
        const T *yp = tile + (size_t)ku * rs + t_begin * 8 + rlane;
        for (int left = t_end - t_begin; left > 0;) {
        const int nb = (sizeof(T) == 4 && left > 8) ? 8 : left;
        left -= nb;
        for (int n = nb; n > 0; --n) {
            T v0[NT], v1[NT];
#pragma unroll
            for (int t = 0; t < NT; ++t) {
                if constexpr (sizeof(T) == 4) { const float2 vv = *reinterpret_cast<const float2 *>(zp[t]); v0[t] = vv.x; v1[t] = vv.y; }
                else { v0[t] = zp[t][0]; v1[t] = zp[t][4]; }
                zp[t] += zinc[t];
            }
            if constexpr (YV) {
                T y0, y1;
                if constexpr (sizeof(T) == 4) { const float2 yy = *reinterpret_cast<const float2 *>(yp); y0 = yy.x; y1 = yy.y; }
                else { y0 = yp[0]; y1 = yp[4]; }
                yp += 8;
                xy0 = fma(v0[0], y0, xy0);
                xy1 = fma(v1[0], y1, xy1);
            }
            int p = 0;
#pragma unroll
            for (int ti = 0; ti < NT; ++ti)
#pragma unroll
                for (int tj = ti; tj < NT; ++tj, ++p) {
                    if (ti == 1 && !need11) continue;
                    acc[p][0] = M::mma(v0[ti], v0[tj], acc[p][0]);
                    acc[p][1] = M::mma(v1[ti], v1[tj], acc[p][1]);
                }
        }
        if constexpr (sizeof(T) == 4) {
#pragma unroll
            for (int p = 0; p < NPAIR; ++p) {
#pragma unroll
                for (int r = 0; r < 4; ++r) accd[p][r] += (double)acc[p][0][r] + (double)acc[p][1][r];
                acc[p][0] = acc_t{0, 0, 0, 0}; acc[p][1] = acc_t{0, 0, 0, 0};
            }
            if constexpr (YV) { xyd += (double)xy0 + (double)xy1; xy0 = T(0); xy1 = T(0); }
        }
        }
        if (nbuf == 1) __syncthreads();
    }
    __syncthreads();
    if constexpr (sizeof(T) == 8) {
#pragma unroll
        for (int p = 0; p < NPAIR; ++p)
#pragma unroll
            for (int r = 0; r < 4; ++r) accd[p][r] = acc[p][0][r] + acc[p][1][r];
        if constexpr (YV) xyd = xy0 + xy1;
    }

    if (HAS_W && a.nvalid) {
        if (nfit) atomicAdd(&nfit_s, nfit);
        __syncthreads();
        if (tid == 0) a.nvalid[g] = (double)nfit_s;
    }
    double *part = reinterpret_cast<double *>(tile0);
    if constexpr (YV) {
        double xy = xyd;
        xy += __shfl_xor(xy, 16);
        xy += __shfl_xor(xy, 32);
        if (lane < 16) part[NPAIR * 4 * 256 + wave * 16 + lane] = xy;
    }
#pragma unroll
    for (int p = 0; p < NPAIR; ++p) {
#pragma unroll
        for (int r = 0; r < 4; ++r) part[(p * 4 + wave) * 256 + r * 64 + lane] = accd[p][r];
    }
    __syncthreads();
    double *G = a.gram + (size_t)g * NZ * NZ;
    const int r = tid >> 6, l = tid & 63;
    const int drow = (sizeof(T) == 4) ? (l >> 4) * 4 + r : (l >> 4) + 4 * r;
    const int dcol = l & 15;
    int p = 0;
#pragma unroll
    for (int ti = 0; ti < NT; ++ti)
#pragma unroll
        for (int tj = ti; tj < NT; ++tj, ++p) {
            double v = 0.0;
#pragma unroll
            for (int w = 0; w < 4; ++w) v += part[(p * 4 + w) * 256 + tid];
            const int i = 16 * ti + drow, j = 16 * tj + dcol;
            if (i < NZ && j < NZ) {
                if (!HAS_W && icpt && i == kt - 1 && j == kt - 1) v = (double)(e - s);
                G[i * NZ + j] = v;
                if (ti != tj) G[j * NZ + i] = v;
            }
        }
    if constexpr (YV) {
        if (tid < 16) {
            double v = 0.0;
#pragma unroll
            for (int w = 0; w < 4; ++w) v += part[NPAIR * 4 * 256 + w * 16 + tid];
            G[tid * NZ + kt] = v;
            G[kt * NZ + tid] = v;
        }
        if (tid == 16) G[kt * NZ + kt] = 0.0;
    }
}

template <typename T, int NT, bool HAS_W, bool YV = false>
static int gram_stream_launch_t(pols_ctx *ctx, const GramArgs &a) {
    const int ncols = a.k_user + 1 + (HAS_W ? 1 : 0);
    int cr = KG_CR;
    if (!ctx->opt.kg_single_buffer)
        while ((size_t)cr * 2 * sizeof(T) <= 4096 && (size_t)ncols * k1m_row_stride<T>(cr * 2) * sizeof(T) <= 48 * 1024) cr *= 2;
    const int rs = k1m_row_stride<T>(cr);
    const int npair = NT * (NT + 1) / 2;
    const int tile_elems = std::max(ncols * rs, (int)((npair * 4 * 256 + (YV ? 64 : 0)) * (sizeof(double) / sizeof(T))));
    const int nbuf = (!ctx->opt.kg_single_buffer && sizeof(T) * (size_t)tile_elems <= 24 * 1024) ? 2 : 1;
    const size_t lds = sizeof(T) * ((size_t)nbuf * tile_elems + 2 * K1M_CONST_ELEMS);
    static OncePerDevice attr_once;
    if (attr_once.needed(ctx->device)) {
        POLS_HIP(hipFuncSetAttribute(reinterpret_cast<const void *>(&gram_stream_kernel<T, NT, HAS_W, YV>),
                                     hipFuncAttributeMaxDynamicSharedMemorySize, 128 * 1024));
        attr_once.done(ctx->device);
    }
    char name[96];
    std::snprintf(name, sizeof(name), "k5_gram_stream_%s_nt%d%s%s_k%d", sizeof(T) == 4 ? "f32" : "f64", NT, HAS_W ? "_w" : "", YV ? "_yv" : "", a.kt);
    ctx->last_kernel = name;
    hipEvent_t ev0, ev1;
    if (timing_pair(ctx, &ev0, &ev1))
        hipExtLaunchKernelGGL((gram_stream_kernel<T, NT, HAS_W, YV>), dim3((unsigned)a.n_groups), dim3(256), (unsigned)lds, ctx->stream, ev0, ev1, 0, a, rs, ncols, tile_elems, nbuf, cr);
    else
        hipLaunchKernelGGL((gram_stream_kernel<T, NT, HAS_W, YV>), dim3((unsigned)a.n_groups), dim3(256), lds, ctx->stream, a, rs, ncols, tile_elems, nbuf, cr);
    POLS_HIP(hipGetLastError());
    return POLS_OK;
}

template <int NW>
__global__ void __launch_bounds__(64 * NW) gram_reduce_kernel(const GramReduceArgs a) {
    __shared__ double part[NW][64];
    const int64_t g = blockIdx.x;
    const int lane = threadIdx.x & 63, wave = threadIdx.x >> 6;
    int v0 = a.first[g], v1 = a.first[g + 1];
    const int nz_ = (int)gridDim.z, z = (int)blockIdx.z;
    if (nz_ > 1) {
        const int per_z = (v1 - v0 + nz_ - 1) / nz_;
        v0 = v0 + z * per_z < v1 ? v0 + z * per_z : v1;
        v1 = v0 + per_z < v1 ? v0 + per_z : v1;
    }
    const int per = (v1 - v0 + NW - 1) / NW, va = v0 + wave * per < v1 ? v0 + wave * per : v1, vb = va + per < v1 ? va + per : v1;
    const int e = blockIdx.y * 64 + lane;
    double acc = 0.0;
    if (e < a.nz2) {
        const double *p = a.part + e;
        int v = va;
        for (; v + 8 <= vb; v += 8) {
            double t[8];
#pragma unroll
            for (int i = 0; i < 8; ++i) t[i] = p[(size_t)(v + i) * a.nz2];
            acc += ((t[0] + t[1]) + (t[2] + t[3])) + ((t[4] + t[5]) + (t[6] + t[7]));
        }
        for (; v < vb; ++v) acc += p[(size_t)v * a.nz2];
    }
    part[wave][lane] = acc;
    __syncthreads();
    if (wave == 0 && e < a.nz2) {
        double t = part[0][lane];
#pragma unroll
        for (int w = 1; w < NW; ++w) t += part[w][lane];
        if (nz_ > 1) a.slices[((size_t)g * nz_ + z) * a.nz2 + e] = t;
        else a.gram[(size_t)g * a.nz2 + e] = t;
    }
    if (a.nvalid && blockIdx.y == 0 && z == 0 && wave == 0) {
        double n = 0.0;
        for (int v = a.first[g] + lane; v < a.first[g + 1]; v += 64) n += a.nv_part[v];
        n = wave_sum_row3(n);
        if (lane == 63) a.nvalid[g] = n;
    }
}

__global__ void __launch_bounds__(64) gram_reduce_final_kernel(const GramReduceArgs a, const int n_slices) {
    const int64_t g = blockIdx.x;
    const int e = blockIdx.y * 64 + threadIdx.x;
    if (e >= a.nz2) return;
    const double *p = a.slices + (size_t)g * n_slices * a.nz2 + e;
    double t = p[0];
    for (int z = 1; z < n_slices; ++z) t += p[(size_t)z * a.nz2];
    a.gram[(size_t)g * a.nz2 + e] = t;
}

int gram_reduce_launch(pols_ctx *ctx, const GramReduceArgs &a) {
    if (a.n_groups == 0) return POLS_OK;
    const unsigned eb = (unsigned)((a.nz2 + 63) / 64);
    if (a.slices && a.n_slices > 1) {
        hipLaunchKernelGGL(gram_reduce_kernel<4>, dim3((unsigned)a.n_groups, eb, (unsigned)a.n_slices), dim3(256), 0, ctx->stream, a);
        hipLaunchKernelGGL(gram_reduce_final_kernel, dim3((unsigned)a.n_groups, eb), dim3(64), 0, ctx->stream, a, a.n_slices);
    } else if (a.max_segments >= 256) {
        hipLaunchKernelGGL(gram_reduce_kernel<16>, dim3((unsigned)a.n_groups, eb), dim3(1024), 0, ctx->stream, a);
    } else {
        hipLaunchKernelGGL(gram_reduce_kernel<4>, dim3((unsigned)a.n_groups, eb), dim3(256), 0, ctx->stream, a);
    }
    POLS_HIP(hipGetLastError());
    return POLS_OK;
}

int gram_stream_launch(pols_ctx *ctx, int dtype, const GramArgs &a) {
    if (gram_valu_takes(ctx, dtype, a)) return gram_valu_launch(ctx, dtype, a);
    if (a.kt + 1 > 32) return fail(POLS_ERR_UNSUPPORTED, "gram_stream: %d features (incl. intercept) > 31", a.kt);
    const bool two = a.kt + 1 > 16, w = a.w != nullptr || a.null_policy != POLS_NULL_IGNORE;
    if (a.kt == 16 && !ctx->opt.kg_noyv) {
        if (dtype == POLS_F32) return w ? gram_stream_launch_t<float, 1, true, true>(ctx, a) : gram_stream_launch_t<float, 1, false, true>(ctx, a);
        return w ? gram_stream_launch_t<double, 1, true, true>(ctx, a) : gram_stream_launch_t<double, 1, false, true>(ctx, a);
    }
    if (dtype == POLS_F32) {
        if (two) return w ? gram_stream_launch_t<float, 2, true>(ctx, a) : gram_stream_launch_t<float, 2, false>(ctx, a);
        return w ? gram_stream_launch_t<float, 1, true>(ctx, a) : gram_stream_launch_t<float, 1, false>(ctx, a);
    }
    if (two) return w ? gram_stream_launch_t<double, 2, true>(ctx, a) : gram_stream_launch_t<double, 2, false>(ctx, a);
    return w ? gram_stream_launch_t<double, 1, true>(ctx, a) : gram_stream_launch_t<double, 1, false>(ctx, a);
}

constexpr int CD_KMAX = 31;

__device__ __forceinline__ double soft_threshold(double x, double thr, bool positive) {
    const double mag = fmax(fabs(x) - thr, 0.0);
    double r = copysign(mag, x);
    if (positive) r = fmax(r, 0.0);
    return r;
}

template <typename T, int LPG>
__global__ void __launch_bounds__(64) gram_cd_kernel(const CdArgs a) {
    constexpr int CD_KMAX = LPG;
    const int lane = threadIdx.x, sub = lane & (LPG - 1);
    const int64_t grp = (int64_t)blockIdx.x * (64 / LPG) + (lane / LPG);
    const bool live = grp < a.n_groups;
    const int kt = a.kt, NZ = kt + 1;
    const int64_t gi = live ? grp : 0;
    const double *G = a.gram + (size_t)gi * NZ * NZ;
    const double n = a.nvalid ? a.nvalid[gi] : (double)(a.offs[gi + 1] - a.offs[gi]);

    double col[CD_KMAX], w[CD_KMAX], b[CD_KMAX], diag[CD_KMAX];
#pragma unroll
    for (int i = 0; i < CD_KMAX; ++i) {
        const bool in = i < kt;
        col[i] = (in && sub < kt) ? G[i * NZ + sub] : 0.0;
        b[i] = in ? G[i * NZ + kt] : 0.0;
        diag[i] = in ? G[i * NZ + i] : 1.0;
        w[i] = 0.0;
    }
    const double alpha_n = a.alpha * n;
    const double thr = alpha_n * a.l1_ratio, l2 = alpha_n * (1.0 - a.l1_ratio);
    const bool positive = a.positive != 0, active_set = a.active_set != 0;
    double wme = 0.0;
    unsigned mask = (kt >= 32) ? 0xffffffffu : ((1u << kt) - 1u);
    bool done = !live || n == 0.0;
    int status = (n == 0.0) ? POLS_GROUP_EMPTY : POLS_GROUP_NOT_CONVERGED;

    for (int64_t it = 0; it < a.max_iter; ++it) {
        if (__all(done)) break;
        double d2 = 0.0;
        const unsigned sweep = mask;
#pragma unroll
        for (int j = 0; j < CD_KMAX; ++j) {
            if (j >= kt) break;
            if (!((sweep >> j) & 1u)) continue;
            double sdot = row_allreduce(col[j] * wme);
            if (LPG == 32) sdot += __shfl_xor(sdot, 16);
            const double dot = b[j] - sdot + diag[j] * w[j];
            const double wn = soft_threshold(dot, thr, positive) / (diag[j] + l2);
            if (!done) {
                const double dw = wn - w[j];
                d2 += dw * dw;
                w[j] = wn;
                if (sub == j) wme = wn;
                if (active_set && fabs(wn) < a.tol) mask &= ~(1u << j);
            }
        }
        if (!done && sqrt(d2) < a.tol) { done = true; status = POLS_GROUP_OK; }
    }
    if (live) {
        if (sub < kt) {
            const double out = (n == 0.0) ? 0.0 : wme;
            if (a.coef) static_cast<T *>(a.coef)[grp * kt + sub] = (T)out;
            if (a.coef64) a.coef64[grp * kt + sub] = out;
        }
        if (sub == 0 && a.status) a.status[grp] = status;
    }
}

int gram_cd_launch(pols_ctx *ctx, int dtype, const CdArgs &a) {
    if (a.kt > CD_KMAX) return fail(POLS_ERR_UNSUPPORTED, "elastic net: %d features (incl. intercept) > %d", a.kt, CD_KMAX);
    if (a.kt <= 16) {
        const unsigned blocks = (unsigned)((a.n_groups + 3) / 4);
        if (dtype == POLS_F32) hipLaunchKernelGGL((gram_cd_kernel<float, 16>), dim3(blocks), dim3(64), 0, ctx->stream, a);
        else hipLaunchKernelGGL((gram_cd_kernel<double, 16>), dim3(blocks), dim3(64), 0, ctx->stream, a);
    } else {
        const unsigned blocks = (unsigned)((a.n_groups + 1) / 2);
        if (dtype == POLS_F32) hipLaunchKernelGGL((gram_cd_kernel<float, 32>), dim3(blocks), dim3(64), 0, ctx->stream, a);
        else hipLaunchKernelGGL((gram_cd_kernel<double, 32>), dim3(blocks), dim3(64), 0, ctx->stream, a);
    }
    POLS_HIP(hipGetLastError());
    return POLS_OK;
}

constexpr int GS_KMAX = 31;

template <typename T>
__global__ void __launch_bounds__(256) gram_solve_kernel(const CdArgs a) {
    __shared__ double Ls[4][GS_KMAX * GS_KMAX];
    __shared__ double rs[4][GS_KMAX];
    const int lane = threadIdx.x & 63, wv = threadIdx.x >> 6;
    const int64_t grp = (int64_t)blockIdx.x * 4 + wv;
    if (grp >= a.n_groups) return;
    const int kt = a.kt, NZ = kt + 1;
    const double *G = a.gram + (size_t)grp * NZ * NZ;
    double *L = Ls[wv];
    double *rinv = rs[wv];
    const int64_t gid = a.glist ? (int64_t)a.glist[grp] : grp;
    const int64_t n = a.nvalid ? (int64_t)a.nvalid[grp] : a.offs[gid + 1] - a.offs[gid];
    for (int q = lane; q < kt * kt; q += 64) {
        const int i = q / kt, j = q - i * kt;
        L[q] = G[i * NZ + j] + (i == j ? a.alpha : 0.0);
    }
    double bi = (lane < kt) ? G[lane * NZ + kt] : 0.0;
    __builtin_amdgcn_wave_barrier();
    bool ok = true;
    for (int j = 0; j < kt && a.solver != 1; ++j) {
        double d = L[j * kt + j];
        const double gjj = d;
        for (int p = 0; p < j; ++p) d -= L[j * kt + p] * L[j * kt + p];
        ok = ok && (d > a.pivot_tol * gjj);
        const double ri = 1.0 / sqrt(d);
        if (lane == 0) rinv[j] = ri;
        if (lane > j && lane < kt) {
            double sacc = L[lane * kt + j];
            for (int p = 0; p < j; ++p) sacc -= L[lane * kt + p] * L[j * kt + p];
            L[lane * kt + j] = sacc * ri;
        }
        __builtin_amdgcn_wave_barrier();
    }
    for (int p = 0; p < kt; ++p) {
        if (lane == p) bi *= rinv[p];
        const double tp = __shfl(bi, p);
        if (lane > p && lane < kt) bi -= L[lane * kt + p] * tp;
    }
    for (int p = kt - 1; p >= 0; --p) {
        if (lane == p) bi *= rinv[p];
        const double bp = __shfl(bi, p);
        if (lane < p) bi -= L[p * kt + lane] * bp;
    }
    if (a.solver == 1 || (!ok && a.lu_fallback)) {
        for (int q = lane; q < kt * kt; q += 64) {
            const int i = q / kt, j = q - i * kt;
            L[q] = G[i * NZ + j] + (i == j ? a.alpha : 0.0);
        }
        bi = (lane < kt) ? G[lane * NZ + kt] : 0.0;
        __builtin_amdgcn_wave_barrier();
        ok = true;
        for (int j = 0; j < kt; ++j) {
            double v = (lane >= j && lane < kt) ? fabs(L[lane * kt + j]) : -1.0;
            int idx = lane;
#pragma unroll
            for (int off = 16; off >= 1; off >>= 1) {
                const double ov = __shfl_xor(v, off);
                const int oi = __shfl_xor(idx, off);
                if (ov > v || (ov == v && oi < idx)) { v = ov; idx = oi; }
            }
            const int pr = __shfl(idx, 0);
            const double piv = L[pr * kt + j];
            ok = ok && (fabs(piv) > 0.0);
            const double bj = __shfl(bi, j), bp = __shfl(bi, pr);
            if (pr != j) {
                if (lane >= j && lane < kt) { const double t = L[j * kt + lane]; L[j * kt + lane] = L[pr * kt + lane]; L[pr * kt + lane] = t; }
                if (lane == j) bi = bp;
                if (lane == pr) bi = bj;
            }
            __builtin_amdgcn_wave_barrier();
            const double brow = __shfl(bi, j);
            if (lane > j && lane < kt) {
                const double f = L[lane * kt + j] / piv;
                for (int c = j + 1; c < kt; ++c) L[lane * kt + c] = fma(-f, L[j * kt + c], L[lane * kt + c]);
                bi = fma(-f, brow, bi);
            }
            __builtin_amdgcn_wave_barrier();
        }
        for (int p = kt - 1; p >= 0; --p) {
            if (lane == p) bi /= L[p * kt + p];
            const double bp = __shfl(bi, p);
            if (lane < p) bi = fma(-L[lane * kt + p], bp, bi);
        }
        ok = ok && __all(lane >= kt || ((bi == bi) && fabs(bi) <= 1.7e308));
    }
    int st = POLS_GROUP_OK;
    if (n == 0) { bi = 0.0; st = POLS_GROUP_EMPTY; }
    else if (!ok) { st = POLS_GROUP_FALLBACK; if (lane == 0 && a.fb_flag) *a.fb_flag = a.epoch; }
    if (lane < kt) {
        if (a.coef) static_cast<T *>(a.coef)[gid * kt + lane] = (T)bi;
        if (a.coef64) a.coef64[grp * kt + lane] = bi;
    }
    if (lane == 0 && a.status) a.status[gid] = st;
}

int gram_solve_launch(pols_ctx *ctx, int dtype, const CdArgs &a) {
    if (a.kt > GS_KMAX) return fail(POLS_ERR_UNSUPPORTED, "%d features (incl. intercept) > %d", a.kt, GS_KMAX);
    const unsigned blocks = (unsigned)((a.n_groups + 3) / 4);
    if (dtype == POLS_F32) hipLaunchKernelGGL(gram_solve_kernel<float>, dim3(blocks), dim3(256), 0, ctx->stream, a);
    else hipLaunchKernelGGL(gram_solve_kernel<double>, dim3(blocks), dim3(256), 0, ctx->stream, a);
    POLS_HIP(hipGetLastError());
    return POLS_OK;
}

template <typename T, int JB>
__global__ void __launch_bounds__(256) predict_kernel(const PredictArgs a) {
    using V = typename Vec16<T>::type;
    constexpr int VEC = Vec16<T>::N;
    const int64_t g = blockIdx.x;
    const int64_t s = a.offs_pairs ? a.offs[2 * g] : a.offs[g], e = a.offs_pairs ? a.offs[2 * g + 1] : a.offs[g + 1];
    const int64_t base = s - (s % VEC);
    const int ku = a.k_user, kt = a.kt;
    const bool icpt = ku != kt;
    const double *cg = a.coef64 ? a.coef64 + (size_t)(a.gmap ? a.gmap[g] : g) * kt : nullptr;
    const T *crow = static_cast<const T *>(a.coef_rows);
    T *pred = static_cast<T *>(a.pred);
    T *resid = static_cast<T *>(a.resid);
    const int pol = a.null_policy;
    for (int64_t row0 = base + ((int64_t)blockIdx.y * 256 + threadIdx.x) * VEC; row0 < e; row0 += (int64_t)gridDim.y * 256 * VEC) {
        const bool full = (row0 >= s) && (row0 + VEC <= e);
        T p[VEC], sw[VEC], yv[VEC];
#pragma unroll
        for (int v = 0; v < VEC; ++v) { p[v] = T(0); sw[v] = T(1); yv[v] = T(0); }
        if (a.w) {
#pragma unroll
            for (int v = 0; v < VEC; ++v) { const int64_t r = row0 + v; if (r >= s && r < e) sw[v] = sqrt(static_cast<const T *>(a.w)[r]); }
        }
        for (int j0 = 0; j0 < kt; j0 += JB) {
            T xb[JB][VEC];
            T cb[JB];
            if (cg) {
#pragma unroll
                for (int u = 0; u < JB; ++u) cb[u] = (j0 + u < kt) ? (T)cg[j0 + u] : T(0);
            }
            if (full) {
                V tv[JB];
#pragma unroll
                for (int u = 0; u < JB; ++u)
                    if (j0 + u < ku) tv[u] = *reinterpret_cast<const V *>(static_cast<const T *>(a.x[j0 + u]) + row0);
#pragma unroll
                for (int u = 0; u < JB; ++u)
#pragma unroll
                    for (int v = 0; v < VEC; ++v) xb[u][v] = (j0 + u < ku) ? vget<T>(tv[u], v) : T(1);
            } else {
#pragma unroll
                for (int u = 0; u < JB; ++u)
#pragma unroll
                    for (int v = 0; v < VEC; ++v) {
                        const int64_t r = row0 + v;
                        xb[u][v] = (j0 + u < ku) ? ((r >= s && r < e) ? static_cast<const T *>(a.x[j0 + u])[r] : T(0)) : T(1);
                    }
            }
#pragma unroll
            for (int u = 0; u < JB; ++u) {
                const int j = j0 + u;
                if (j < kt) {
#pragma unroll
                    for (int v = 0; v < VEC; ++v) {
                        const int64_t r = row0 + v;
                        T c;
                        if (cg) c = cb[u];
                        else c = (r >= s && r < e) ? crow[r * kt + j] : T(0);
                        p[v] = fma(null_fill<T>(pol, xb[u][v]) * sw[v], c, p[v]);
                    }
                }
            }
        }
        (void)icpt;
        if (a.w) {
#pragma unroll
            for (int v = 0; v < VEC; ++v) p[v] *= T(1) / sw[v];
        }
        if (resid || pol == POLS_NULL_DROP) {
#pragma unroll
            for (int v = 0; v < VEC; ++v) { const int64_t r = row0 + v; if (r >= s && r < e) yv[v] = static_cast<const T *>(a.y)[r]; }
        }
        if (pol == POLS_NULL_DROP) {
            unsigned dropped = 0;
#pragma unroll
            for (int v = 0; v < VEC; ++v) {
                const int64_t r = row0 + v;
                if (r >= s && r < e && !null_row_in_fit<T>(pol, a.valid, a.y, a.x, ku, r)) dropped |= 1u << v;
            }
#pragma unroll
            for (int v = 0; v < VEC; ++v) p[v] = nan_if<T>((dropped >> v) & 1u, p[v]);
        }
        if (full) {
            if (pred) { V o; if constexpr (VEC == 4) o = V{p[0], p[1], p[2], p[3]}; else o = V{p[0], p[1]}; store_stream(reinterpret_cast<V *>(pred + row0), o); }
            if (resid) {
                V o;
                if constexpr (VEC == 4) o = V{yv[0] - p[0], yv[1] - p[1], yv[2] - p[2], yv[3] - p[3]}; else o = V{yv[0] - p[0], yv[1] - p[1]};
                store_stream(reinterpret_cast<V *>(resid + row0), o);
            }
        } else {
#pragma unroll
            for (int v = 0; v < VEC; ++v) {
                const int64_t r = row0 + v;
                if (r >= s && r < e) { if (pred) pred[r] = p[v]; if (resid) resid[r] = yv[v] - p[v]; }
            }
        }
    }
}

template <typename T, int JB, bool HAS_W = false, bool DROP = false>
__global__ void __launch_bounds__(256) predict_groups_kernel(const PredictArgs a) {
    using V = typename Vec16<T>::type;
    constexpr int VEC = Vec16<T>::N;
    const int64_t g = blockIdx.x;
    const int64_t s = a.offs_pairs ? a.offs[2 * g] : a.offs[g], e = a.offs_pairs ? a.offs[2 * g + 1] : a.offs[g + 1];
    const int64_t base = s - (s % VEC);
    const int ku = a.k_user, kt = a.kt;
    const double *cg = a.coef64 + (size_t)(a.gmap ? a.gmap[g] : g) * kt;
    T *pred = static_cast<T *>(a.pred);
    T *resid = static_cast<T *>(a.resid);
    const int pol = a.null_policy;
    T c[JB];
#pragma unroll
    for (int u = 0; u < JB; ++u) c[u] = (u < kt) ? (T)cg[u] : T(0);
    for (int64_t row0 = base + ((int64_t)blockIdx.y * 256 + threadIdx.x) * VEC; row0 < e; row0 += (int64_t)gridDim.y * 256 * VEC) {
        T p[VEC];
#pragma unroll
        for (int v = 0; v < VEC; ++v) p[v] = T(0);
        if ((row0 >= s) && (row0 + VEC <= e)) {
            V tv[JB];
#pragma unroll
            for (int u = 0; u < JB; ++u)
                if (u < ku) tv[u] = *reinterpret_cast<const V *>(static_cast<const T *>(a.x[u]) + row0);
            T sw[VEC];
#pragma unroll
            for (int v = 0; v < VEC; ++v) sw[v] = T(1);
            if constexpr (HAS_W) {
                const V wv = *reinterpret_cast<const V *>(static_cast<const T *>(a.w) + row0);
#pragma unroll
                for (int v = 0; v < VEC; ++v) sw[v] = sqrt(vget<T>(wv, v));
            }
#pragma unroll
            for (int u = 0; u < JB; ++u)
#pragma unroll
                for (int v = 0; v < VEC; ++v) {
                    const T xv = (u < ku) ? null_fill<T>(pol, vget<T>(tv[u], v)) : T(1);
                    p[v] = fma(HAS_W ? xv * sw[v] : xv, c[u], p[v]);
                }
            if constexpr (HAS_W) {
#pragma unroll
                for (int v = 0; v < VEC; ++v) p[v] *= T(1) / sw[v];
            }
            V yv;
            if (DROP || resid) yv = *reinterpret_cast<const V *>(static_cast<const T *>(a.y) + row0);
            if constexpr (DROP) {
#pragma unroll
                for (int v = 0; v < VEC; ++v) {
                    const T y1 = vget<T>(yv, v);
                    bool fit = (y1 == y1) && !(a.valid && !a.valid[row0 + v]);
#pragma unroll
                    for (int u = 0; u < JB; ++u)
                        if (u < ku) { const T x1 = vget<T>(tv[u], v); fit = fit && (x1 == x1); }
                    p[v] = nan_if<T>(fit ? 0u : 1u, p[v]);
                }
            }
            if (pred) {
                V o;
                if constexpr (VEC == 4) o = V{p[0], p[1], p[2], p[3]}; else o = V{p[0], p[1]};
                store_stream(reinterpret_cast<V *>(pred + row0), o);
            }
            if (resid) {
                V o;
                if constexpr (VEC == 4) o = V{yv.x - p[0], yv.y - p[1], yv.z - p[2], yv.w - p[3]}; else o = V{yv.x - p[0], yv.y - p[1]};
                store_stream(reinterpret_cast<V *>(resid + row0), o);
            }
        } else {
#pragma unroll
            for (int v = 0; v < VEC; ++v) {
                const int64_t r = row0 + v;
                if (r >= s && r < e) {
                    const T sw = HAS_W ? sqrt(static_cast<const T *>(a.w)[r]) : T(1);
#pragma unroll
                    for (int u = 0; u < JB; ++u) {
                        const T xv = (u < ku) ? null_fill<T>(pol, static_cast<const T *>(a.x[u])[r]) : T(1);
                        p[v] = fma(HAS_W ? xv * sw : xv, c[u], p[v]);
                    }
                    if constexpr (HAS_W) p[v] *= T(1) / sw;
                    if constexpr (DROP) p[v] = nan_if<T>(null_row_in_fit<T>(pol, a.valid, a.y, a.x, ku, r) ? 0u : 1u, p[v]);
                    if (pred) pred[r] = p[v];
                    if (resid) resid[r] = static_cast<const T *>(a.y)[r] - p[v];
                }
            }
        }
    }
}

int predict_launch(pols_ctx *ctx, int dtype, const PredictArgs &a) {
    if (a.n_groups == 0) return POLS_OK;
    const int64_t per_wg = 256 * (dtype == POLS_F32 ? 4 : 2);
    int64_t gy = std::max<int64_t>(1, (a.max_item_rows + per_wg - 1) / per_wg);
    gy = std::min<int64_t>(std::min<int64_t>(gy, 1024), std::max<int64_t>(1, 16384 / a.n_groups));
    if (ctx->opt.predict_loop) gy = 1;
    const dim3 grid((unsigned)a.n_groups, (unsigned)gy);
    const int jb = a.kt <= 4 ? 4 : (a.kt <= 8 ? 8 : (a.kt <= 12 ? 12 : 16));
    if (a.coef64 && (a.pred || a.resid) && ((a.null_policy != POLS_NULL_DROP && !a.resid) || a.y) && a.kt <= 16 && !ctx->opt.predict_loop) {
#define POLS_PREDICT_GROUPS_GO(T, W, D)                                                                                     \
    do {                                                                                                                    \
        if (jb == 4) hipLaunchKernelGGL((predict_groups_kernel<T, 4, W, D>), grid, dim3(256), 0, ctx->stream, a);           \
        else if (jb == 8) hipLaunchKernelGGL((predict_groups_kernel<T, 8, W, D>), grid, dim3(256), 0, ctx->stream, a);      \
        else if (jb == 12) hipLaunchKernelGGL((predict_groups_kernel<T, 12, W, D>), grid, dim3(256), 0, ctx->stream, a);    \
        else hipLaunchKernelGGL((predict_groups_kernel<T, 16, W, D>), grid, dim3(256), 0, ctx->stream, a);                  \
    } while (0)
#define POLS_PREDICT_GROUPS_T(T)                                                                                            \
    do {                                                                                                                    \
        if (a.null_policy == POLS_NULL_DROP) { if (a.w) POLS_PREDICT_GROUPS_GO(T, true, true); else POLS_PREDICT_GROUPS_GO(T, false, true); } \
        else { if (a.w) POLS_PREDICT_GROUPS_GO(T, true, false); else POLS_PREDICT_GROUPS_GO(T, false, false); }            \
    } while (0)
        if (dtype == POLS_F32) POLS_PREDICT_GROUPS_T(float);
        else POLS_PREDICT_GROUPS_T(double);
#undef POLS_PREDICT_GROUPS_T
#undef POLS_PREDICT_GROUPS_GO
        POLS_HIP(hipGetLastError());
        return POLS_OK;
    }
#define POLS_PREDICT_GO(T)                                                                                          \
    do {                                                                                                            \
        if (jb == 4) hipLaunchKernelGGL((predict_kernel<T, 4>), grid, dim3(256), 0, ctx->stream, a);                \
        else if (jb <= 8) hipLaunchKernelGGL((predict_kernel<T, 8>), grid, dim3(256), 0, ctx->stream, a);           \
        else hipLaunchKernelGGL((predict_kernel<T, 16>), grid, dim3(256), 0, ctx->stream, a);                       \
    } while (0)
    if (dtype == POLS_F32) POLS_PREDICT_GO(float);
    else POLS_PREDICT_GO(double);
#undef POLS_PREDICT_GO
    POLS_HIP(hipGetLastError());
    return POLS_OK;
}

}
```

### polars_ols_amd/csrc/k5_enet.hpp

```cpp
#pragma once
#include "common.hpp"

namespace pols {

struct GramArgs {
    const void *y;
    const void *w;
    const void *x[POLS_MAX_FEATURES];
    const int64_t *offs;
    int64_t n_groups;
    int64_t n_rows;
    double *gram;
    int32_t k_user;
    int32_t kt;
    const uint8_t *valid;
    int32_t null_policy;
    double *nvalid;
    int32_t offs_pairs;
};

struct CdArgs {
    const double *gram;
    const int64_t *offs;
    int64_t n_groups;
    void *coef;
    double *coef64;
    int32_t *status;
    double alpha, l1_ratio, tol;
    double pivot_tol;
    int32_t *fb_flag;
    int32_t epoch;
    int64_t max_iter;
    int32_t positive, active_set, kt;
    const double *nvalid;
    int32_t solver;
    int32_t lu_fallback;
    const int32_t *glist;
};

struct PredictArgs {
    const void *y;
    const void *w;
    const void *x[POLS_MAX_FEATURES];
    const int64_t *offs;
    int64_t n_groups;
    int64_t n_rows;
    const double *coef64;
    const void *coef_rows;
    void *pred;
    void *resid;
    int32_t k_user, kt;
    const uint8_t *valid;
    int32_t null_policy;
    const int32_t *gmap;
    int64_t max_item_rows;
    int32_t offs_pairs;
};

struct GramReduceArgs {
    const double *part;
    const double *nv_part;
    const int32_t *first;
    double *gram;
    double *nvalid;
    int64_t n_groups;
    int32_t nz2;
    int32_t max_segments;
    double *slices;
    int32_t n_slices;
};
int gram_reduce_launch(pols_ctx *ctx, const GramReduceArgs &a);

int gram_stream_launch(pols_ctx *ctx, int dtype, const GramArgs &a);
constexpr int K5V_MAX_KT = 10;
constexpr int K5V_MAX_KT_F32 = 13;
bool gram_valu_takes(const pols_ctx *ctx, int dtype, const GramArgs &a);
int gram_valu_launch(pols_ctx *ctx, int dtype, const GramArgs &a);
int gram_cd_launch(pols_ctx *ctx, int dtype, const CdArgs &a);
int gram_solve_launch(pols_ctx *ctx, int dtype, const CdArgs &a);
int predict_launch(pols_ctx *ctx, int dtype, const PredictArgs &a);

}
```

### polars_ols_amd/csrc/k5v_gram.hip

```cpp
#include "k5_enet.hpp"

namespace pols {

__device__ __forceinline__ void k5v_scale(float4 &z, const float (&sw)[4]) { z.x *= sw[0]; z.y *= sw[1]; z.z *= sw[2]; z.w *= sw[3]; }
__device__ __forceinline__ void k5v_scale(double2 &z, const double (&sw)[2]) { z.x *= sw[0]; z.y *= sw[1]; }

template <int NZ>
__host__ __device__ constexpr int k5v_tri(int i, int j) { return i * NZ - i * (i - 1) / 2 + (j - i); }

template <typename T, int KT, bool HAS_W, bool NULLS>
__global__ void __launch_bounds__(256) gram_valu_kernel(const GramArgs a) {
    using V = typename Vec16<T>::type;
    constexpr int VEC = Vec16<T>::N;
    constexpr int NZ = KT + 1, NACC = NZ * (NZ + 1) / 2;
    const int tid = threadIdx.x, lane = tid & 63, wave = tid >> 6;
    const int64_t g = blockIdx.x;
    const int64_t s = a.offs_pairs ? a.offs[2 * g] : a.offs[g], e = a.offs_pairs ? a.offs[2 * g + 1] : a.offs[g + 1];
    const int64_t base = s - (s % VEC);
    const int ku = a.k_user;

    T acc[NACC];
#pragma unroll
    for (int q = 0; q < NACC; ++q) acc[q] = T(0);
    const int pol = a.null_policy;
    int nfit = 0;

    constexpr int SL = 32, NSL = (NACC + SL - 1) / SL;
    __shared__ double part[4][NSL * SL];
    for (int q = lane; q < NSL * SL; q += 64) part[wave][q] = 0.0;
    auto flush = [&]() {
#pragma unroll
        for (int sl = 0; sl < NSL; ++sl) {
            double accd[SL];
#pragma unroll
            for (int q = 0; q < SL; ++q) accd[q] = (sl * SL + q < NACC) ? (double)acc[(sl * SL + q < NACC) ? sl * SL + q : 0] : 0.0;
            double u[SL / 4];
            wave_reduce_scatter<double, SL>(accd, u);
            if ((lane & 15) == 0) {
                const int r = rs_perm(lane >> 4);
#pragma unroll
                for (int i = 0; i < SL / 4; ++i) part[wave][sl * SL + 4 * i + r] += u[i];
            }
        }
#pragma unroll
        for (int q = 0; q < NACC; ++q) acc[q] = T(0);
    };
    constexpr int K5V_FLUSH_STEPS = 32;
    int since = 0;

    const int64_t n_steps = (e - base + 256 * VEC - 1) / (256 * VEC);
    for (int64_t it = 0; it < n_steps; ++it) {
        const int64_t row0 = base + (it * 256 + tid) * VEC;
        if constexpr (sizeof(T) == 4) {
            if (since == K5V_FLUSH_STEPS) { flush(); since = 0; }
            ++since;
        }
        if (row0 >= e) continue;
        V z[NZ];
        if (row0 >= s && row0 + VEC <= e) {
#pragma unroll
            for (int j = 0; j < KT; ++j) {
                if (j < KT - 1 || j < ku) z[j] = load_stream(reinterpret_cast<const V *>(static_cast<const T *>(a.x[j]) + row0));
                else { if constexpr (VEC == 4) z[j] = V{T(1), T(1), T(1), T(1)}; else z[j] = V{T(1), T(1)}; }
            }
            z[KT] = load_stream(reinterpret_cast<const V *>(static_cast<const T *>(a.y) + row0));
            if constexpr (HAS_W || NULLS) {
                T sw[VEC];
#pragma unroll
                for (int v = 0; v < VEC; ++v) sw[v] = T(1);
                if constexpr (HAS_W) {
                    const V wv = load_stream(reinterpret_cast<const V *>(static_cast<const T *>(a.w) + row0));
#pragma unroll
                    for (int v = 0; v < VEC; ++v) sw[v] = sqrt(vget<T>(wv, v));
                }
                if constexpr (NULLS) {
                    bool ok[VEC];
#pragma unroll
                    for (int v = 0; v < VEC; ++v) ok[v] = true;
                    if (a.valid && null_checks_y(pol)) {
#pragma unroll
                        for (int v = 0; v < VEC; ++v) ok[v] = a.valid[row0 + v] != 0;
                    }
                    if (null_checks_y(pol)) {
#pragma unroll
                        for (int v = 0; v < VEC; ++v) { const T yv = vget<T>(z[KT], v); ok[v] = ok[v] && (yv == yv); }
                    }
                    if (null_checks_x(pol)) {
#pragma unroll
                        for (int j = 0; j < KT; ++j)
#pragma unroll
                            for (int v = 0; v < VEC; ++v) { const T xv = vget<T>(z[j], v); ok[v] = ok[v] && (xv == xv); }
                    }
#pragma unroll
                    for (int v = 0; v < VEC; ++v) { nfit += ok[v] ? 1 : 0; sw[v] = ok[v] ? sw[v] : T(0); }
#pragma unroll
                    for (int j = 0; j < NZ; ++j) {
                        T t[VEC];
#pragma unroll
                        for (int v = 0; v < VEC; ++v) t[v] = ok[v] ? null_fill<T>(pol, vget<T>(z[j], v)) : T(0);
                        if constexpr (VEC == 4) z[j] = V{t[0], t[1], t[2], t[3]}; else z[j] = V{t[0], t[1]};
                    }
                }
#pragma unroll
                for (int j = 0; j < NZ; ++j) k5v_scale(z[j], sw);
            }
        } else {
#pragma unroll
            for (int j = 0; j < NZ; ++j) {
                T t[VEC];
#pragma unroll
                for (int v = 0; v < VEC; ++v) {
                    const int64_t r = row0 + v;
                    const bool in = r >= s && r < e;
                    if (j == KT) t[v] = in ? static_cast<const T *>(a.y)[r] : T(0);
                    else if (j < KT - 1 || j < ku) t[v] = in ? static_cast<const T *>(a.x[j])[r] : T(0);
                    else t[v] = in ? T(1) : T(0);
                    bool use = in;
                    if constexpr (NULLS) {
                        use = in && null_row_in_fit<T>(pol, a.valid, a.y, a.x, ku, r);
                        t[v] = use ? null_fill<T>(pol, t[v]) : T(0);
                        if (j == KT) nfit += use ? 1 : 0;
                    }
                    if constexpr (HAS_W) t[v] = use ? t[v] * sqrt(static_cast<const T *>(a.w)[r]) : T(0);
                }
                if constexpr (VEC == 4) z[j] = V{t[0], t[1], t[2], t[3]}; else z[j] = V{t[0], t[1]};
            }
        }
#pragma unroll
        for (int v = 0; v < VEC; ++v)
#pragma unroll
            for (int i = 0; i < NZ; ++i) {
                const T zi = vget<T>(z[i], v);
#pragma unroll
                for (int j = i; j < NZ; ++j) acc[k5v_tri<NZ>(i, j)] = fma(zi, vget<T>(z[j], v), acc[k5v_tri<NZ>(i, j)]);
            }
    }

    flush();
    __shared__ int nfit_s;
    if constexpr (NULLS) { if (tid == 0) nfit_s = 0; }
    __syncthreads();
    if constexpr (NULLS) {
        if (nfit) atomicAdd(&nfit_s, nfit);
        __syncthreads();
        if (tid == 0 && a.nvalid) a.nvalid[g] = (double)nfit_s;
    }
    double *G = a.gram + (size_t)g * NZ * NZ;
    for (int t = tid; t < NZ * NZ; t += 256) {
        const int i = t / NZ, j = t - i * NZ;
        const int lo = i < j ? i : j, hi = i < j ? j : i;
        const int q = lo * NZ - lo * (lo - 1) / 2 + (hi - lo);
        G[t] = ((part[0][q] + part[1][q]) + part[2][q]) + part[3][q];
    }
}

template <typename T, int KT, bool HAS_W, bool NULLS>
static void k5v_go_w(pols_ctx *ctx, const GramArgs &a) {
    hipEvent_t ev0, ev1;
    if (timing_pair(ctx, &ev0, &ev1)) hipExtLaunchKernelGGL((gram_valu_kernel<T, KT, HAS_W, NULLS>), dim3((unsigned)a.n_groups), dim3(256), 0, ctx->stream, ev0, ev1, 0, a);
    else hipLaunchKernelGGL((gram_valu_kernel<T, KT, HAS_W, NULLS>), dim3((unsigned)a.n_groups), dim3(256), 0, ctx->stream, a);
}
template <typename T, int KT>
static void k5v_go(pols_ctx *ctx, const GramArgs &a) {
    const bool nulls = a.null_policy != POLS_NULL_IGNORE;
    if (a.w) { if (nulls) k5v_go_w<T, KT, true, true>(ctx, a); else k5v_go_w<T, KT, true, false>(ctx, a); }
    else { if (nulls) k5v_go_w<T, KT, false, true>(ctx, a); else k5v_go_w<T, KT, false, false>(ctx, a); }
}

template <typename T>
static int k5v_launch_t(pols_ctx *ctx, const GramArgs &a) {
    switch (a.kt) {
        case 1: k5v_go<T, 1>(ctx, a); break;
        case 2: k5v_go<T, 2>(ctx, a); break;
        case 3: k5v_go<T, 3>(ctx, a); break;
        case 4: k5v_go<T, 4>(ctx, a); break;
        case 5: k5v_go<T, 5>(ctx, a); break;
        case 6: k5v_go<T, 6>(ctx, a); break;
        case 7: k5v_go<T, 7>(ctx, a); break;
        case 8: k5v_go<T, 8>(ctx, a); break;
        case 9: k5v_go<T, 9>(ctx, a); break;
        case 10: k5v_go<T, 10>(ctx, a); break;
        default:
            if constexpr (sizeof(T) == 4) {
                switch (a.kt) {
                    case 11: k5v_go<T, 11>(ctx, a); break;
                    case 12: k5v_go<T, 12>(ctx, a); break;
                    case 13: k5v_go<T, 13>(ctx, a); break;
                    default: return fail(POLS_ERR_UNSUPPORTED, "k5v: %d columns", a.kt);
                }
                break;
            }
            return fail(POLS_ERR_UNSUPPORTED, "k5v: %d columns", a.kt);
    }
    POLS_HIP(hipGetLastError());
    return POLS_OK;
}

bool gram_valu_takes(const pols_ctx *ctx, int dtype, const GramArgs &a) {
    return a.kt >= 1 && a.kt <= (dtype == POLS_F32 ? K5V_MAX_KT_F32 : K5V_MAX_KT) && (a.null_policy == POLS_NULL_IGNORE ? !a.nvalid : a.nvalid != nullptr) && !ctx->opt.kg_single_buffer;
}

int gram_valu_launch(pols_ctx *ctx, int dtype, const GramArgs &a) {
    if (a.n_groups > 0x7ffffff0LL) return fail(POLS_ERR_UNSUPPORTED, "too many groups for one launch");
    char name[96];
    std::snprintf(name, sizeof(name), "k5_gram_stream_%s_valu%s%s_k%d", dtype == POLS_F32 ? "f32" : "f64", a.w ? "_w" : "", a.null_policy != POLS_NULL_IGNORE ? "_nulls" : "", a.kt);
    ctx->last_kernel = name;
    return dtype == POLS_F32 ? k5v_launch_t<float>(ctx, a) : k5v_launch_t<double>(ctx, a);
}

}
```

Measured before the change: 130.1 million.

## Fuse gram reduce and solve into gram stream kernel via per-group tickets

For small group counts on the streaming gram path, the segment reduction and the per-group Cholesky/LU solve now run as a tail inside the gram stream kernel. The last block to finish a group, found through an atomic ticket counter, does the reduction and solve. This removes one or two extra kernel launches and the round trip of the gram matrices through global memory between them. The cost is a larger LDS reservation, more template instantiations, and a persistent ticket buffer that must be reset correctly between calls.

```diff
diff --git a/polars_ols_amd/csrc/api.hip b/polars_ols_amd/csrc/api.hip
--- a/polars_ols_amd/csrc/api.hip
+++ b/polars_ols_amd/csrc/api.hip
@@ -196,6 +196,7 @@
     else if (ieq(key, "PREDICT_LOOP")) o.predict_loop = on;
     else if (ieq(key, "K2_NOPREFETCH")) o.k2_noprefetch = on;
     else if (ieq(key, "NO_SPLIT")) o.no_split = on;
+    else if (ieq(key, "STREAM_UNFUSED")) o.stream_unfused = on;
     else if (ieq(key, "K1_PASSES")) o.k1_passes = on ? std::atoi(v) : d.k1_passes;
     else if (ieq(key, "K1_WG")) o.k1_wg = on ? std::atoi(v) : d.k1_wg;
     else if (ieq(key, "K1T_RC4")) o.k1t_rc4 = on ? (std::atoi(v) != 0) : d.k1t_rc4;
@@ -226,7 +227,7 @@
     static const char *const keys[] = {"TIMELINE", "K1_NOOCC4", "K1_NOFAST", "K1_NOTINY", "K1_NORC1", "K1_SHAPE", "K1_F64_TEAM",
                                        "KG_NOYV", "K2_NOPREFETCH", "K1_PASSES", "K1_WG", "RLS_SPINS", "RLS_EARLY", "K1T_RC4", "K1_NT_LOADS", "STATIC_ENGINE",
                                        "RLS_ENGINE", "RLM_ENGINE", "GLM_ENGINE", "ROLLING_ENGINE", "K1_ENGINE", "K9_TAKE", "K1_PERSIST", "K1_PERSIST_SUB", "K1T_SUB32", "K1_NOEDGE", "K1T_SUB8",
-                                       "K1_XCD", "NO_SPLIT", "DEBUG_SKIP_FIXUP", "K4P_LPS", "SEG_TARGET", "K1_RC2_WIDE", "KG_SINGLE_BUFFER", "PREDICT_LOOP", "NO_CLASSES"};
+                                       "K1_XCD", "NO_SPLIT", "STREAM_UNFUSED", "DEBUG_SKIP_FIXUP", "K4P_LPS", "SEG_TARGET", "K1_RC2_WIDE", "KG_SINGLE_BUFFER", "PREDICT_LOOP", "NO_CLASSES"};
     char name[64];
     for (const char *k : keys) {
         std::snprintf(name, sizeof(name), "POLS_%s", k);
@@ -1093,18 +1094,15 @@
         ga.gram = split ? gram_part : static_cast<double *>(scr);
         ga.k_user = b->n_features; ga.kt = kt;
         ga.valid = st.valid; ga.null_policy = pol; ga.nvalid = split ? nv_part : nvalid;
-        if ((rc = gram_stream_launch(ctx, b->dtype, ga))) return rc;
+        GramReduceArgs ra;
+        std::memset(&ra, 0, sizeof(ra));
         if (split) {
-            GramReduceArgs ra;
-            std::memset(&ra, 0, sizeof(ra));
             ra.part = gram_part; ra.nv_part = nv_part; ra.first = seg_first;
             ra.gram = static_cast<double *>(scr); ra.nvalid = nvalid; ra.n_groups = ng; ra.nz2 = (int32_t)(nz * nz);
             ra.max_segments = (int32_t)std::min<int64_t>(1 << 30, sg.max_seg);
             if (n_slices > 1) { ra.slices = reinterpret_cast<double *>(static_cast<char *>(scr) + gram_bytes + c64_bytes + nv_bytes); ra.n_slices = n_slices; }
-            if ((rc = gram_reduce_launch(ctx, ra))) return rc;
-            ga.gram = static_cast<double *>(scr);
-            ctx->last_kernel += "_split";
-        }
+        }
+        const bool fused = !enet && !ids && n_slices == 1 && !ctx->opt.stream_unfused && (split ? (ng <= 256 && sg.max_seg < 256) : ng <= 64);
         CdArgs ca;
         std::memset(&ca, 0, sizeof(ca));
         ca.gram = ga.gram; ca.offs = d_offs; ca.n_groups = ng; ca.glist = d_ids;
@@ -1113,15 +1111,33 @@
         ca.alpha = alpha; ca.l1_ratio = enet_l1; ca.tol = p->tol; ca.max_iter = p->max_iter;
         ca.positive = positive ? 1 : 0; ca.active_set = (m == POLS_SOLVE_CD_ACTIVE_SET) ? 1 : 0; ca.kt = kt;
         ca.nvalid = nvalid;
-        if (enet) {
-            if ((rc = gram_cd_launch(ctx, b->dtype, ca))) return rc;
-        } else {
+        if (!enet) {
             ca.alpha = ridge_alpha;
             ca.solver = (m == POLS_SOLVE_LU) ? 1 : 0;
             ca.lu_fallback = (!ols_branch && m != POLS_SOLVE_SVD) ? 1 : 0;
             ca.pivot_tol = ca.lu_fallback ? chol_noise : pivot_tol;
             ca.fb_flag = ctx->fb_flag; ca.epoch = ctx->epoch;
-            if ((rc = gram_solve_launch(ctx, b->dtype, ca))) return rc;
+        }
+        if (fused) {
+            void *tk = nullptr;
+            bool fresh = false;
+            if ((rc = grow(ctx->work[(int)Work::StreamTickets], sizeof(int32_t) * (size_t)ng, &tk, &fresh))) return rc;
+            if (fresh) POLS_HIP(hipMemsetAsync(tk, 0, ctx->work[(int)Work::StreamTickets].cap, ctx->stream));
+            GramTailArgs tl;
+            std::memset(&tl, 0, sizeof(tl));
+            tl.tickets = static_cast<int32_t *>(tk); tl.seg_map = split ? seg_map : nullptr;
+            tl.red = ra; tl.solve = ca;
+            if (split) tl.solve.gram = ra.gram;
+            if ((rc = gram_stream_launch(ctx, b->dtype, ga, &tl))) return rc;
+        } else {
+            if ((rc = gram_stream_launch(ctx, b->dtype, ga))) return rc;
+            if (split && (rc = gram_reduce_launch(ctx, ra))) return rc;
+        }
+        if (split) { ga.gram = static_cast<double *>(scr); ctx->last_kernel += "_split"; }
+        if (!fused) {
+            ca.gram = ga.gram;
+            if (enet) { if ((rc = gram_cd_launch(ctx, b->dtype, ca))) return rc; }
+            else if ((rc = gram_solve_launch(ctx, b->dtype, ca))) return rc;
         }
         if (st.pred || st.resid) {
             PredictArgs pa;
diff --git a/polars_ols_amd/csrc/common.hpp b/polars_ols_amd/csrc/common.hpp
--- a/polars_ols_amd/csrc/common.hpp
+++ b/polars_ols_amd/csrc/common.hpp
@@ -87,6 +87,7 @@
     IvState,
     IvInputs,
     IvOut,
+    StreamTickets,
     Count
 };
 
@@ -119,6 +120,7 @@
     int k9_take = 0;
     int k1_nt_loads = -1;
     bool no_split = false;
+    bool stream_unfused = false;
     bool k2_noprefetch = false;
     bool k1_noedge = false;
     int k1t_sub32 = -1;
diff --git a/polars_ols_amd/csrc/k5_enet.hip b/polars_ols_amd/csrc/k5_enet.hip
--- a/polars_ols_amd/csrc/k5_enet.hip
+++ b/polars_ols_amd/csrc/k5_enet.hip
@@ -1,12 +1,13 @@
 #include "k5_enet.hpp"
 #include "k1m_kernel.inl"
+#include "k5_tail.inl"
 
 namespace pols {
 
 constexpr int KG_CR = 256;
 
-template <typename T, int NT, bool HAS_W, bool YV = false>
-__global__ void __launch_bounds__(256) gram_stream_kernel(const GramArgs a, const int rs, const int ncols, const int tile_elems, const int nbuf, const int cr) {
+template <typename T, int NT, bool HAS_W, bool YV = false, bool FUSED = false>
+__global__ void __launch_bounds__(256) gram_stream_kernel(const GramArgs a, const int rs, const int ncols, const int tile_elems, const int nbuf, const int cr, const GramTailOf<FUSED> tl) {
     using V = typename Vec16<T>::type;
     using M = Mfma16<T>;
     using acc_t = typename M::acc_t;
@@ -242,33 +243,43 @@
         }
         if (tid == 16) G[kt * NZ + kt] = 0.0;
     }
+    if constexpr (FUSED) gram_tail<T>(tl.t, g, reinterpret_cast<double *>(tile0));
 }
 
 template <typename T, int NT, bool HAS_W, bool YV = false>
-static int gram_stream_launch_t(pols_ctx *ctx, const GramArgs &a) {
+static int gram_stream_launch_t(pols_ctx *ctx, const GramArgs &a, const GramTailArgs *tail) {
     const int ncols = a.k_user + 1 + (HAS_W ? 1 : 0);
     int cr = KG_CR;
     if (!ctx->opt.kg_single_buffer)
         while ((size_t)cr * 2 * sizeof(T) <= 4096 && (size_t)ncols * k1m_row_stride<T>(cr * 2) * sizeof(T) <= 48 * 1024) cr *= 2;
     const int rs = k1m_row_stride<T>(cr);
     const int npair = NT * (NT + 1) / 2;
-    const int tile_elems = std::max(ncols * rs, (int)((npair * 4 * 256 + (YV ? 64 : 0)) * (sizeof(double) / sizeof(T))));
+    const int tile_elems = std::max(ncols * rs, (int)(std::max(npair * 4 * 256 + (YV ? 64 : 0), tail ? GRAM_TAIL_LDS : 0) * (sizeof(double) / sizeof(T))));
     const int nbuf = (!ctx->opt.kg_single_buffer && sizeof(T) * (size_t)tile_elems <= 24 * 1024) ? 2 : 1;
     const size_t lds = sizeof(T) * ((size_t)nbuf * tile_elems + 2 * K1M_CONST_ELEMS);
     static OncePerDevice attr_once;
     if (attr_once.needed(ctx->device)) {
-        POLS_HIP(hipFuncSetAttribute(reinterpret_cast<const void *>(&gram_stream_kernel<T, NT, HAS_W, YV>),
+        POLS_HIP(hipFuncSetAttribute(reinterpret_cast<const void *>(&gram_stream_kernel<T, NT, HAS_W, YV, false>),
+                                     hipFuncAttributeMaxDynamicSharedMemorySize, 128 * 1024));
+        POLS_HIP(hipFuncSetAttribute(reinterpret_cast<const void *>(&gram_stream_kernel<T, NT, HAS_W, YV, true>),
                                      hipFuncAttributeMaxDynamicSharedMemorySize, 128 * 1024));
         attr_once.done(ctx->device);
     }
     char name[96];
-    std::snprintf(name, sizeof(name), "k5_gram_stream_%s_nt%d%s%s_k%d", sizeof(T) == 4 ? "f32" : "f64", NT, HAS_W ? "_w" : "", YV ? "_yv" : "", a.kt);
+    std::snprintf(name, sizeof(name), "k5_gram_stream_%s_nt%d%s%s_k%d%s", sizeof(T) == 4 ? "f32" : "f64", NT, HAS_W ? "_w" : "", YV ? "_yv" : "", a.kt,
+                  tail ? "_solve_fused" : "");
     ctx->last_kernel = name;
     hipEvent_t ev0, ev1;
-    if (timing_pair(ctx, &ev0, &ev1))
-        hipExtLaunchKernelGGL((gram_stream_kernel<T, NT, HAS_W, YV>), dim3((unsigned)a.n_groups), dim3(256), (unsigned)lds, ctx->stream, ev0, ev1, 0, a, rs, ncols, tile_elems, nbuf, cr);
+    const bool timed = timing_pair(ctx, &ev0, &ev1);
+    if (tail) {
+        GramTailOf<true> tl;
+        tl.t = *tail;
+        if (timed) hipExtLaunchKernelGGL((gram_stream_kernel<T, NT, HAS_W, YV, true>), dim3((unsigned)a.n_groups), dim3(256), (unsigned)lds, ctx->stream, ev0, ev1, 0, a, rs, ncols, tile_elems, nbuf, cr, tl);
+        else hipLaunchKernelGGL((gram_stream_kernel<T, NT, HAS_W, YV, true>), dim3((unsigned)a.n_groups), dim3(256), lds, ctx->stream, a, rs, ncols, tile_elems, nbuf, cr, tl);
+    } else if (timed)
+        hipExtLaunchKernelGGL((gram_stream_kernel<T, NT, HAS_W, YV, false>), dim3((unsigned)a.n_groups), dim3(256), (unsigned)lds, ctx->stream, ev0, ev1, 0, a, rs, ncols, tile_elems, nbuf, cr, GramTailOf<false>());
     else
-        hipLaunchKernelGGL((gram_stream_kernel<T, NT, HAS_W, YV>), dim3((unsigned)a.n_groups), dim3(256), lds, ctx->stream, a, rs, ncols, tile_elems, nbuf, cr);
+        hipLaunchKernelGGL((gram_stream_kernel<T, NT, HAS_W, YV, false>), dim3((unsigned)a.n_groups), dim3(256), lds, ctx->stream, a, rs, ncols, tile_elems, nbuf, cr, GramTailOf<false>());
     POLS_HIP(hipGetLastError());
     return POLS_OK;
 }
@@ -276,44 +287,7 @@
 template <int NW>
 __global__ void __launch_bounds__(64 * NW) gram_reduce_kernel(const GramReduceArgs a) {
     __shared__ double part[NW][64];
-    const int64_t g = blockIdx.x;
-    const int lane = threadIdx.x & 63, wave = threadIdx.x >> 6;
-    int v0 = a.first[g], v1 = a.first[g + 1];
-    const int nz_ = (int)gridDim.z, z = (int)blockIdx.z;
-    if (nz_ > 1) {
-        const int per_z = (v1 - v0 + nz_ - 1) / nz_;
-        v0 = v0 + z * per_z < v1 ? v0 + z * per_z : v1;
-        v1 = v0 + per_z < v1 ? v0 + per_z : v1;
-    }
-    const int per = (v1 - v0 + NW - 1) / NW, va = v0 + wave * per < v1 ? v0 + wave * per : v1, vb = va + per < v1 ? va + per : v1;
-    const int e = blockIdx.y * 64 + lane;
-    double acc = 0.0;
-    if (e < a.nz2) {
-        const double *p = a.part + e;
-        int v = va;
-        for (; v + 8 <= vb; v += 8) {
-            double t[8];
-#pragma unroll
-            for (int i = 0; i < 8; ++i) t[i] = p[(size_t)(v + i) * a.nz2];
-            acc += ((t[0] + t[1]) + (t[2] + t[3])) + ((t[4] + t[5]) + (t[6] + t[7]));
-        }
-        for (; v < vb; ++v) acc += p[(size_t)v * a.nz2];
-    }
-    part[wave][lane] = acc;
-    __syncthreads();
-    if (wave == 0 && e < a.nz2) {
-        double t = part[0][lane];
-#pragma unroll
-        for (int w = 1; w < NW; ++w) t += part[w][lane];
-        if (nz_ > 1) a.slices[((size_t)g * nz_ + z) * a.nz2 + e] = t;
-        else a.gram[(size_t)g * a.nz2 + e] = t;
-    }
-    if (a.nvalid && blockIdx.y == 0 && z == 0 && wave == 0) {
-        double n = 0.0;
-        for (int v = a.first[g] + lane; v < a.first[g + 1]; v += 64) n += a.nv_part[v];
-        n = wave_sum_row3(n);
-        if (lane == 63) a.nvalid[g] = n;
-    }
+    gram_reduce_block<NW>(a, blockIdx.x, (int)blockIdx.y, (int)blockIdx.z, (int)gridDim.z, part);
 }
 
 __global__ void __launch_bounds__(64) gram_reduce_final_kernel(const GramReduceArgs a, const int n_slices) {
@@ -341,20 +315,20 @@
     return POLS_OK;
 }
 
-int gram_stream_launch(pols_ctx *ctx, int dtype, const GramArgs &a) {
-    if (gram_valu_takes(ctx, dtype, a)) return gram_valu_launch(ctx, dtype, a);
+int gram_stream_launch(pols_ctx *ctx, int dtype, const GramArgs &a, const GramTailArgs *tail) {
+    if (gram_valu_takes(ctx, dtype, a)) return tail ? gram_valu_fused_launch(ctx, dtype, a, *tail) : gram_valu_launch(ctx, dtype, a);
     if (a.kt + 1 > 32) return fail(POLS_ERR_UNSUPPORTED, "gram_stream: %d features (incl. intercept) > 31", a.kt);
     const bool two = a.kt + 1 > 16, w = a.w != nullptr || a.null_policy != POLS_NULL_IGNORE;
     if (a.kt == 16 && !ctx->opt.kg_noyv) {
-        if (dtype == POLS_F32) return w ? gram_stream_launch_t<float, 1, true, true>(ctx, a) : gram_stream_launch_t<float, 1, false, true>(ctx, a);
-        return w ? gram_stream_launch_t<double, 1, true, true>(ctx, a) : gram_stream_launch_t<double, 1, false, true>(ctx, a);
+        if (dtype == POLS_F32) return w ? gram_stream_launch_t<float, 1, true, true>(ctx, a, tail) : gram_stream_launch_t<float, 1, false, true>(ctx, a, tail);
+        return w ? gram_stream_launch_t<double, 1, true, true>(ctx, a, tail) : gram_stream_launch_t<double, 1, false, true>(ctx, a, tail);
     }
     if (dtype == POLS_F32) {
-        if (two) return w ? gram_stream_launch_t<float, 2, true>(ctx, a) : gram_stream_launch_t<float, 2, false>(ctx, a);
-        return w ? gram_stream_launch_t<float, 1, true>(ctx, a) : gram_stream_launch_t<float, 1, false>(ctx, a);
-    }
-    if (two) return w ? gram_stream_launch_t<double, 2, true>(ctx, a) : gram_stream_launch_t<double, 2, false>(ctx, a);
-    return w ? gram_stream_launch_t<double, 1, true>(ctx, a) : gram_stream_launch_t<double, 1, false>(ctx, a);
+        if (two) return w ? gram_stream_launch_t<float, 2, true>(ctx, a, tail) : gram_stream_launch_t<float, 2, false>(ctx, a, tail);
+        return w ? gram_stream_launch_t<float, 1, true>(ctx, a, tail) : gram_stream_launch_t<float, 1, false>(ctx, a, tail);
+    }
+    if (two) return w ? gram_stream_launch_t<double, 2, true>(ctx, a, tail) : gram_stream_launch_t<double, 2, false>(ctx, a, tail);
+    return w ? gram_stream_launch_t<double, 1, true>(ctx, a, tail) : gram_stream_launch_t<double, 1, false>(ctx, a, tail);
 }
 
 constexpr int CD_KMAX = 31;
@@ -441,102 +415,14 @@
     return POLS_OK;
 }
 
-constexpr int GS_KMAX = 31;
-
 template <typename T>
 __global__ void __launch_bounds__(256) gram_solve_kernel(const CdArgs a) {
     __shared__ double Ls[4][GS_KMAX * GS_KMAX];
     __shared__ double rs[4][GS_KMAX];
-    const int lane = threadIdx.x & 63, wv = threadIdx.x >> 6;
+    const int wv = threadIdx.x >> 6;
     const int64_t grp = (int64_t)blockIdx.x * 4 + wv;
     if (grp >= a.n_groups) return;
-    const int kt = a.kt, NZ = kt + 1;
-    const double *G = a.gram + (size_t)grp * NZ * NZ;
-    double *L = Ls[wv];
-    double *rinv = rs[wv];
-    const int64_t gid = a.glist ? (int64_t)a.glist[grp] : grp;
-    const int64_t n = a.nvalid ? (int64_t)a.nvalid[grp] : a.offs[gid + 1] - a.offs[gid];
-    for (int q = lane; q < kt * kt; q += 64) {
-        const int i = q / kt, j = q - i * kt;
-        L[q] = G[i * NZ + j] + (i == j ? a.alpha : 0.0);
-    }
-    double bi = (lane < kt) ? G[lane * NZ + kt] : 0.0;
-    __builtin_amdgcn_wave_barrier();
-    bool ok = true;
-    for (int j = 0; j < kt && a.solver != 1; ++j) {
-        double d = L[j * kt + j];
-        const double gjj = d;
-        for (int p = 0; p < j; ++p) d -= L[j * kt + p] * L[j * kt + p];
-        ok = ok && (d > a.pivot_tol * gjj);
-        const double ri = 1.0 / sqrt(d);
-        if (lane == 0) rinv[j] = ri;
-        if (lane > j && lane < kt) {
-            double sacc = L[lane * kt + j];
-            for (int p = 0; p < j; ++p) sacc -= L[lane * kt + p] * L[j * kt + p];
-            L[lane * kt + j] = sacc * ri;
-        }
-        __builtin_amdgcn_wave_barrier();
-    }
-    for (int p = 0; p < kt; ++p) {
-        if (lane == p) bi *= rinv[p];
-        const double tp = __shfl(bi, p);
-        if (lane > p && lane < kt) bi -= L[lane * kt + p] * tp;
-    }
-    for (int p = kt - 1; p >= 0; --p) {
-        if (lane == p) bi *= rinv[p];
-        const double bp = __shfl(bi, p);
-        if (lane < p) bi -= L[p * kt + lane] * bp;
-    }
-    if (a.solver == 1 || (!ok && a.lu_fallback)) {
-        for (int q = lane; q < kt * kt; q += 64) {
-            const int i = q / kt, j = q - i * kt;
-            L[q] = G[i * NZ + j] + (i == j ? a.alpha : 0.0);
-        }
-        bi = (lane < kt) ? G[lane * NZ + kt] : 0.0;
-        __builtin_amdgcn_wave_barrier();
-        ok = true;
-        for (int j = 0; j < kt; ++j) {
-            double v = (lane >= j && lane < kt) ? fabs(L[lane * kt + j]) : -1.0;
-            int idx = lane;
-#pragma unroll
-            for (int off = 16; off >= 1; off >>= 1) {
-                const double ov = __shfl_xor(v, off);
-                const int oi = __shfl_xor(idx, off);
-                if (ov > v || (ov == v && oi < idx)) { v = ov; idx = oi; }
-            }
-            const int pr = __shfl(idx, 0);
-            const double piv = L[pr * kt + j];
-            ok = ok && (fabs(piv) > 0.0);
-            const double bj = __shfl(bi, j), bp = __shfl(bi, pr);
-            if (pr != j) {
-                if (lane >= j && lane < kt) { const double t = L[j * kt + lane]; L[j * kt + lane] = L[pr * kt + lane]; L[pr * kt + lane] = t; }
-                if (lane == j) bi = bp;
-                if (lane == pr) bi = bj;
-            }
-            __builtin_amdgcn_wave_barrier();
-            const double brow = __shfl(bi, j);
-            if (lane > j && lane < kt) {
-                const double f = L[lane * kt + j] / piv;
-                for (int c = j + 1; c < kt; ++c) L[lane * kt + c] = fma(-f, L[j * kt + c], L[lane * kt + c]);
-                bi = fma(-f, brow, bi);
-            }
-            __builtin_amdgcn_wave_barrier();
-        }
-        for (int p = kt - 1; p >= 0; --p) {
-            if (lane == p) bi /= L[p * kt + p];
-            const double bp = __shfl(bi, p);
-            if (lane < p) bi = fma(-L[lane * kt + p], bp, bi);
-        }
-        ok = ok && __all(lane >= kt || ((bi == bi) && fabs(bi) <= 1.7e308));
-    }
-    int st = POLS_GROUP_OK;
-    if (n == 0) { bi = 0.0; st = POLS_GROUP_EMPTY; }
-    else if (!ok) { st = POLS_GROUP_FALLBACK; if (lane == 0 && a.fb_flag) *a.fb_flag = a.epoch; }
-    if (lane < kt) {
-        if (a.coef) static_cast<T *>(a.coef)[gid * kt + lane] = (T)bi;
-        if (a.coef64) a.coef64[grp * kt + lane] = bi;
-    }
-    if (lane == 0 && a.status) a.status[gid] = st;
+    gram_solve_wave<T>(a, grp, Ls[wv], rs[wv]);
 }
 
 int gram_solve_launch(pols_ctx *ctx, int dtype, const CdArgs &a) {
diff --git a/polars_ols_amd/csrc/k5_enet.hpp b/polars_ols_amd/csrc/k5_enet.hpp
--- a/polars_ols_amd/csrc/k5_enet.hpp
+++ b/polars_ols_amd/csrc/k5_enet.hpp
@@ -71,11 +71,22 @@
 };
 int gram_reduce_launch(pols_ctx *ctx, const GramReduceArgs &a);
 
-int gram_stream_launch(pols_ctx *ctx, int dtype, const GramArgs &a);
+struct GramTailArgs {
+    int32_t *tickets;
+    const int32_t *seg_map;
+    GramReduceArgs red;
+    CdArgs solve;
+};
+
+template <bool FUSED> struct GramTailOf {};
+template <> struct GramTailOf<true> { GramTailArgs t; };
+
+int gram_stream_launch(pols_ctx *ctx, int dtype, const GramArgs &a, const GramTailArgs *tail = nullptr);
 constexpr int K5V_MAX_KT = 10;
 constexpr int K5V_MAX_KT_F32 = 13;
 bool gram_valu_takes(const pols_ctx *ctx, int dtype, const GramArgs &a);
 int gram_valu_launch(pols_ctx *ctx, int dtype, const GramArgs &a);
+int gram_valu_fused_launch(pols_ctx *ctx, int dtype, const GramArgs &a, const GramTailArgs &tail);
 int gram_cd_launch(pols_ctx *ctx, int dtype, const CdArgs &a);
 int gram_solve_launch(pols_ctx *ctx, int dtype, const CdArgs &a);
 int predict_launch(pols_ctx *ctx, int dtype, const PredictArgs &a);
diff --git a/polars_ols_amd/csrc/k5v_fused.hip b/polars_ols_amd/csrc/k5v_fused.hip
--- /dev/null
+++ b/polars_ols_amd/csrc/k5v_fused.hip
@@ -0,0 +1,15 @@
+#include "k5v_kernel.inl"
+
+namespace pols {
+
+int gram_valu_fused_launch(pols_ctx *ctx, int dtype, const GramArgs &a, const GramTailArgs &tail) {
+    if (a.n_groups > 0x7ffffff0LL) return fail(POLS_ERR_UNSUPPORTED, "too many groups for one launch");
+    char name[96];
+    std::snprintf(name, sizeof(name), "k5_gram_stream_%s_valu%s%s_k%d_solve_fused", dtype == POLS_F32 ? "f32" : "f64", a.w ? "_w" : "", a.null_policy != POLS_NULL_IGNORE ? "_nulls" : "", a.kt);
+    ctx->last_kernel = name;
+    GramTailOf<true> lp;
+    lp.t = tail;
+    return dtype == POLS_F32 ? k5v_launch_t<float>(ctx, a, lp) : k5v_launch_t<double>(ctx, a, lp);
+}
+
+}
diff --git a/polars_ols_amd/csrc/k5v_gram.hip b/polars_ols_amd/csrc/k5v_gram.hip
--- a/polars_ols_amd/csrc/k5v_gram.hip
+++ b/polars_ols_amd/csrc/k5v_gram.hip
@@ -1,200 +1,6 @@
-#include "k5_enet.hpp"
+#include "k5v_kernel.inl"
 
 namespace pols {
-
-__device__ __forceinline__ void k5v_scale(float4 &z, const float (&sw)[4]) { z.x *= sw[0]; z.y *= sw[1]; z.z *= sw[2]; z.w *= sw[3]; }
-__device__ __forceinline__ void k5v_scale(double2 &z, const double (&sw)[2]) { z.x *= sw[0]; z.y *= sw[1]; }
-
-template <int NZ>
-__host__ __device__ constexpr int k5v_tri(int i, int j) { return i * NZ - i * (i - 1) / 2 + (j - i); }
-
-template <typename T, int KT, bool HAS_W, bool NULLS>
-__global__ void __launch_bounds__(256) gram_valu_kernel(const GramArgs a) {
-    using V = typename Vec16<T>::type;
-    constexpr int VEC = Vec16<T>::N;
-    constexpr int NZ = KT + 1, NACC = NZ * (NZ + 1) / 2;
-    const int tid = threadIdx.x, lane = tid & 63, wave = tid >> 6;
-    const int64_t g = blockIdx.x;
-    const int64_t s = a.offs_pairs ? a.offs[2 * g] : a.offs[g], e = a.offs_pairs ? a.offs[2 * g + 1] : a.offs[g + 1];
-    const int64_t base = s - (s % VEC);
-    const int ku = a.k_user;
-
-    T acc[NACC];
-#pragma unroll
-    for (int q = 0; q < NACC; ++q) acc[q] = T(0);
-    const int pol = a.null_policy;
-    int nfit = 0;
-
-    constexpr int SL = 32, NSL = (NACC + SL - 1) / SL;
-    __shared__ double part[4][NSL * SL];
-    for (int q = lane; q < NSL * SL; q += 64) part[wave][q] = 0.0;
-    auto flush = [&]() {
-#pragma unroll
-        for (int sl = 0; sl < NSL; ++sl) {
-            double accd[SL];
-#pragma unroll
-            for (int q = 0; q < SL; ++q) accd[q] = (sl * SL + q < NACC) ? (double)acc[(sl * SL + q < NACC) ? sl * SL + q : 0] : 0.0;
-            double u[SL / 4];
-            wave_reduce_scatter<double, SL>(accd, u);
-            if ((lane & 15) == 0) {
-                const int r = rs_perm(lane >> 4);
-#pragma unroll
-                for (int i = 0; i < SL / 4; ++i) part[wave][sl * SL + 4 * i + r] += u[i];
-            }
-        }
-#pragma unroll
-        for (int q = 0; q < NACC; ++q) acc[q] = T(0);
-    };
-    constexpr int K5V_FLUSH_STEPS = 32;
-    int since = 0;
-
-    const int64_t n_steps = (e - base + 256 * VEC - 1) / (256 * VEC);
-    for (int64_t it = 0; it < n_steps; ++it) {
-        const int64_t row0 = base + (it * 256 + tid) * VEC;
-        if constexpr (sizeof(T) == 4) {
-            if (since == K5V_FLUSH_STEPS) { flush(); since = 0; }
-            ++since;
-        }
-        if (row0 >= e) continue;
-        V z[NZ];
-        if (row0 >= s && row0 + VEC <= e) {
-#pragma unroll
-            for (int j = 0; j < KT; ++j) {
-                if (j < KT - 1 || j < ku) z[j] = load_stream(reinterpret_cast<const V *>(static_cast<const T *>(a.x[j]) + row0));
-                else { if constexpr (VEC == 4) z[j] = V{T(1), T(1), T(1), T(1)}; else z[j] = V{T(1), T(1)}; }
-            }
-            z[KT] = load_stream(reinterpret_cast<const V *>(static_cast<const T *>(a.y) + row0));
-            if constexpr (HAS_W || NULLS) {
-                T sw[VEC];
-#pragma unroll
-                for (int v = 0; v < VEC; ++v) sw[v] = T(1);
-                if constexpr (HAS_W) {
-                    const V wv = load_stream(reinterpret_cast<const V *>(static_cast<const T *>(a.w) + row0));
-#pragma unroll
-                    for (int v = 0; v < VEC; ++v) sw[v] = sqrt(vget<T>(wv, v));
-                }
-                if constexpr (NULLS) {
-                    bool ok[VEC];
-#pragma unroll
-                    for (int v = 0; v < VEC; ++v) ok[v] = true;
-                    if (a.valid && null_checks_y(pol)) {
-#pragma unroll
-                        for (int v = 0; v < VEC; ++v) ok[v] = a.valid[row0 + v] != 0;
-                    }
-                    if (null_checks_y(pol)) {
-#pragma unroll
-                        for (int v = 0; v < VEC; ++v) { const T yv = vget<T>(z[KT], v); ok[v] = ok[v] && (yv == yv); }
-                    }
-                    if (null_checks_x(pol)) {
-#pragma unroll
-                        for (int j = 0; j < KT; ++j)
-#pragma unroll
-                            for (int v = 0; v < VEC; ++v) { const T xv = vget<T>(z[j], v); ok[v] = ok[v] && (xv == xv); }
-                    }
-#pragma unroll
-                    for (int v = 0; v < VEC; ++v) { nfit += ok[v] ? 1 : 0; sw[v] = ok[v] ? sw[v] : T(0); }
-#pragma unroll
-                    for (int j = 0; j < NZ; ++j) {
-                        T t[VEC];
-#pragma unroll
-                        for (int v = 0; v < VEC; ++v) t[v] = ok[v] ? null_fill<T>(pol, vget<T>(z[j], v)) : T(0);
-                        if constexpr (VEC == 4) z[j] = V{t[0], t[1], t[2], t[3]}; else z[j] = V{t[0], t[1]};
-                    }
-                }
-#pragma unroll
-                for (int j = 0; j < NZ; ++j) k5v_scale(z[j], sw);
-            }
-        } else {
-#pragma unroll
-            for (int j = 0; j < NZ; ++j) {
-                T t[VEC];
-#pragma unroll
-                for (int v = 0; v < VEC; ++v) {
-                    const int64_t r = row0 + v;
-                    const bool in = r >= s && r < e;
-                    if (j == KT) t[v] = in ? static_cast<const T *>(a.y)[r] : T(0);
-                    else if (j < KT - 1 || j < ku) t[v] = in ? static_cast<const T *>(a.x[j])[r] : T(0);
-                    else t[v] = in ? T(1) : T(0);
-                    bool use = in;
-                    if constexpr (NULLS) {
-                        use = in && null_row_in_fit<T>(pol, a.valid, a.y, a.x, ku, r);
-                        t[v] = use ? null_fill<T>(pol, t[v]) : T(0);
-                        if (j == KT) nfit += use ? 1 : 0;
-                    }
-                    if constexpr (HAS_W) t[v] = use ? t[v] * sqrt(static_cast<const T *>(a.w)[r]) : T(0);
-                }
-                if constexpr (VEC == 4) z[j] = V{t[0], t[1], t[2], t[3]}; else z[j] = V{t[0], t[1]};
-            }
-        }
-#pragma unroll
-        for (int v = 0; v < VEC; ++v)
-#pragma unroll
-            for (int i = 0; i < NZ; ++i) {
-                const T zi = vget<T>(z[i], v);
-#pragma unroll
-                for (int j = i; j < NZ; ++j) acc[k5v_tri<NZ>(i, j)] = fma(zi, vget<T>(z[j], v), acc[k5v_tri<NZ>(i, j)]);
-            }
-    }
-
-    flush();
-    __shared__ int nfit_s;
-    if constexpr (NULLS) { if (tid == 0) nfit_s = 0; }
-    __syncthreads();
-    if constexpr (NULLS) {
-        if (nfit) atomicAdd(&nfit_s, nfit);
-        __syncthreads();
-        if (tid == 0 && a.nvalid) a.nvalid[g] = (double)nfit_s;
-    }
-    double *G = a.gram + (size_t)g * NZ * NZ;
-    for (int t = tid; t < NZ * NZ; t += 256) {
-        const int i = t / NZ, j = t - i * NZ;
-        const int lo = i < j ? i : j, hi = i < j ? j : i;
-        const int q = lo * NZ - lo * (lo - 1) / 2 + (hi - lo);
-        G[t] = ((part[0][q] + part[1][q]) + part[2][q]) + part[3][q];
-    }
-}
-
-template <typename T, int KT, bool HAS_W, bool NULLS>
-static void k5v_go_w(pols_ctx *ctx, const GramArgs &a) {
-    hipEvent_t ev0, ev1;
-    if (timing_pair(ctx, &ev0, &ev1)) hipExtLaunchKernelGGL((gram_valu_kernel<T, KT, HAS_W, NULLS>), dim3((unsigned)a.n_groups), dim3(256), 0, ctx->stream, ev0, ev1, 0, a);
-    else hipLaunchKernelGGL((gram_valu_kernel<T, KT, HAS_W, NULLS>), dim3((unsigned)a.n_groups), dim3(256), 0, ctx->stream, a);
-}
-template <typename T, int KT>
-static void k5v_go(pols_ctx *ctx, const GramArgs &a) {
-    const bool nulls = a.null_policy != POLS_NULL_IGNORE;
-    if (a.w) { if (nulls) k5v_go_w<T, KT, true, true>(ctx, a); else k5v_go_w<T, KT, true, false>(ctx, a); }
-    else { if (nulls) k5v_go_w<T, KT, false, true>(ctx, a); else k5v_go_w<T, KT, false, false>(ctx, a); }
-}
-
-template <typename T>
-static int k5v_launch_t(pols_ctx *ctx, const GramArgs &a) {
-    switch (a.kt) {
-        case 1: k5v_go<T, 1>(ctx, a); break;
-        case 2: k5v_go<T, 2>(ctx, a); break;
-        case 3: k5v_go<T, 3>(ctx, a); break;
-        case 4: k5v_go<T, 4>(ctx, a); break;
-        case 5: k5v_go<T, 5>(ctx, a); break;
-        case 6: k5v_go<T, 6>(ctx, a); break;
-        case 7: k5v_go<T, 7>(ctx, a); break;
-        case 8: k5v_go<T, 8>(ctx, a); break;
-        case 9: k5v_go<T, 9>(ctx, a); break;
-        case 10: k5v_go<T, 10>(ctx, a); break;
-        default:
-            if constexpr (sizeof(T) == 4) {
-                switch (a.kt) {
-                    case 11: k5v_go<T, 11>(ctx, a); break;
-                    case 12: k5v_go<T, 12>(ctx, a); break;
-                    case 13: k5v_go<T, 13>(ctx, a); break;
-                    default: return fail(POLS_ERR_UNSUPPORTED, "k5v: %d columns", a.kt);
-                }
-                break;
-            }
-            return fail(POLS_ERR_UNSUPPORTED, "k5v: %d columns", a.kt);
-    }
-    POLS_HIP(hipGetLastError());
-    return POLS_OK;
-}
 
 bool gram_valu_takes(const pols_ctx *ctx, int dtype, const GramArgs &a) {
     return a.kt >= 1 && a.kt <= (dtype == POLS_F32 ? K5V_MAX_KT_F32 : K5V_MAX_KT) && (a.null_policy == POLS_NULL_IGNORE ? !a.nvalid : a.nvalid != nullptr) && !ctx->opt.kg_single_buffer;
@@ -205,7 +11,7 @@
     char name[96];
     std::snprintf(name, sizeof(name), "k5_gram_stream_%s_valu%s%s_k%d", dtype == POLS_F32 ? "f32" : "f64", a.w ? "_w" : "", a.null_policy != POLS_NULL_IGNORE ? "_nulls" : "", a.kt);
     ctx->last_kernel = name;
-    return dtype == POLS_F32 ? k5v_launch_t<float>(ctx, a) : k5v_launch_t<double>(ctx, a);
+    return dtype == POLS_F32 ? k5v_launch_t<float>(ctx, a, GramTailOf<false>()) : k5v_launch_t<double>(ctx, a, GramTailOf<false>());
 }
 
 }
```

Result: no change. 129.7 million (-0.3%).
